# johannes-graeter/limo

Hardware: AMD Instinct MI355X
Metric: keyframe-BA window solves/sec (5 KF, ~2k landmarks) (higher is better)
Workload: dtype f64; 1 GPU; C2: KITTI-00-shaped windows, 5 keyframes x 2000 landmarks, LiDAR depth + ground plane, solveTrimmed schedule {2, trim 5%, <=100 LM iterations}; batch_windows_per_gpu=16384, distinct_windows_per_gpu=4096, observations_per_batch=144288124, depth_observations_per_batch=68405568, parallelism=single, converged=16328

## Files before the change

### include/limo_hip.h

```cpp
#ifndef LIMO_HIP_H_
#define LIMO_HIP_H_

#include <stddef.h>
#include <stdint.h>

#ifdef __cplusplus
extern "C" {
#endif

#define LIMO_ABI_VERSION 6

enum limo_fixation { LIMO_FIX_POSE = 0, LIMO_FIX_SCALE = 1, LIMO_FIX_NONE = 2 };

enum limo_status {
    LIMO_OK = 0,
    LIMO_ERR_INVALID = -1,
    LIMO_ERR_NOT_ENOUGH_KF = -2,
    LIMO_ERR_RUNTIME = -3,
    LIMO_ERR_NO_DEVICE = -4,
    LIMO_ERR_UNSUPPORTED = -5
};

enum limo_termination { LIMO_CONVERGENCE = 0, LIMO_NO_CONVERGENCE = 1, LIMO_FAILURE = 2 };

// ... 19 lines not shown
    const int32_t* obs_cam;
    const float* obs_u;
    const float* obs_v;
    const float* obs_d;
} limo_ba_window;

typedef struct limo_ba_options {
    double depth_thres;
    double reprojection_thres;
    double depth_quantile;
    double reprojection_quantile;
    int32_t num_trim_rounds;
    int32_t trim_solver_iterations;
    int32_t min_landmarks_for_trimming;
    int32_t minimum_number_residual_groups;
    int32_t max_num_iterations;
    double max_solver_time_sec;
    double function_tolerance;
    double gradient_tolerance;
    double parameter_tolerance;
    double initial_trust_region_radius;
    double max_trust_region_radius;
    double min_trust_region_radius;
    double min_lm_diagonal;
    double max_lm_diagonal;
    double min_relative_decrease;
    int32_t max_num_consecutive_invalid_steps;
    int32_t jacobi_scaling;
} limo_ba_options;

typedef struct limo_ba_report {
    int32_t termination;
    int32_t num_solves;
    int32_t iterations_total;
    int32_t iterations_final;
    int32_t successful_steps;
    int32_t n_depth_blocks;
    int32_t n_repr_blocks;
    int32_t n_gp_blocks;
    int32_t n_trimmed_landmarks;
    int32_t num_linearizations;
    double initial_cost;
    double final_cost;
    double time_sec;
} limo_ba_report;

typedef struct limo_ctx limo_ctx;
typedef struct limo_ba_batch limo_ba_batch;

int limo_abi_version(void);
int limo_ctx_create(int device, limo_ctx** out);
void limo_ctx_destroy(limo_ctx* ctx);
int limo_ctx_set_stream(limo_ctx* ctx, void* hip_stream);
const char* limo_last_error(const limo_ctx* ctx);
void* limo_host_alloc(size_t bytes);
void limo_host_free(void* p);

void limo_ba_default_options(limo_ba_options* out);

int limo_ba_solve(limo_ctx* ctx, limo_ba_window* window, const limo_ba_options* opts, limo_ba_report* report);

int limo_ba_batch_create(limo_ctx* ctx, int32_t n_windows, const limo_ba_window* windows, limo_ba_batch** out);
int limo_ba_batch_solve(limo_ba_batch* batch, const limo_ba_options* opts);
int limo_ba_batch_reset(limo_ba_batch* batch);
int limo_ba_batch_download(limo_ba_batch* batch, limo_ba_window* windows_out, limo_ba_report* reports);
void limo_ba_batch_destroy(limo_ba_batch* batch);
int limo_ba_batch_trimmed(limo_ba_batch* batch, int32_t window, uint8_t* removed);
int limo_ba_batch_kernel_stats(limo_ba_batch* batch, int reset, double* linearize_ms, int64_t* linearize_launches,
                               double* total_ms);
#define LIMO_KERNEL_LINEARIZE 0
#define LIMO_KERNEL_SCHUR 1
int limo_ba_batch_kernel_time(limo_ba_batch* batch, int kernel, double* ms, int64_t* launches);

#define LIMO_COMM_ID_BYTES 128
int limo_comm_unique_id(unsigned char id[LIMO_COMM_ID_BYTES]);
int limo_ctx_comm_init(limo_ctx* ctx, const unsigned char id[LIMO_COMM_ID_BYTES], int rank, int world);
typedef void (*limo_exchange_fn)(const double* send, double* recv, long long count, int kind, void* user);
int limo_ctx_comm_init_host(limo_ctx* ctx, limo_exchange_fn fn, void* user, int rank, int world);
int limo_ba_solve_sharded(limo_ctx* ctx, limo_ba_window* window, const limo_ba_options* opts, int n_shards,
                          limo_ba_report* report);
int limo_ctx_exchange_stats(limo_ctx* ctx, int64_t* stats3);
int64_t limo_ctx_coop_fallbacks(const limo_ctx* ctx);
int limo_ctx_last_solve_info(const limo_ctx* ctx, int64_t info[8]);

typedef struct limo_ba_iteration {
    int32_t solve;
    int32_t solve_kind;
    int32_t iteration;
    uint8_t step_is_valid, step_is_successful, pad[2];
    double cost;
    double cost_change, gradient_max_norm, step_norm, relative_decrease, trust_region_radius;
} limo_ba_iteration;
int limo_ctx_set_iteration_log(limo_ctx* ctx, int32_t on);
int limo_ba_batch_iteration_log(limo_ba_batch* batch, int32_t window, int32_t cap, limo_ba_iteration* out, int32_t* n);
int limo_ctx_last_iteration_log(limo_ctx* ctx, int32_t window, int32_t cap, limo_ba_iteration* out, int32_t* n);

int limo_ba_evaluate(limo_ctx* ctx, const limo_ba_window* window, const limo_ba_options* opts, int apply_loss,
                     double* cost, double* residuals, double* jac_pose, double* jac_lm, uint8_t* valid);

int limo_ba_evaluate_batch_time(limo_ctx* ctx, int32_t n_windows, const limo_ba_window* windows, const limo_ba_options* opts,
                                int32_t reps, double* device_ms);

typedef struct limo_speed_prior {
    double speed_weight;
    double dt_cur;
    double vel_prev[3];
    double pose_before[7];
} limo_speed_prior;
int limo_ba_adjust_pose_only(limo_ctx* ctx, limo_ba_window* window, const limo_speed_prior* prior,
                             const limo_ba_options* opts, limo_ba_report* report);

int limo_ba_batch_create_pose_only(limo_ctx* ctx, int32_t n_windows, const limo_ba_window* windows,
                                   const limo_speed_prior* priors, limo_ba_batch** out);
int limo_ba_adjust_pose_only_batch(limo_ctx* ctx, int32_t n_windows, limo_ba_window* windows, const limo_speed_prior* priors,
                                   const limo_ba_options* opts, limo_ba_report* reports);

int limo_ba_solve_fixed_landmarks(limo_ctx* ctx, limo_ba_window* window, const uint8_t* lm_fixed, const limo_ba_options* opts,
                                  limo_ba_report* report);
int limo_ba_batch_create_fixed_landmarks(limo_ctx* ctx, int32_t n_windows, const limo_ba_window* windows, const uint8_t* const* lm_fixed,
                                         limo_ba_batch** out);

enum limo_row_kind {
    LIMO_ROW_GROUND_HEIGHT = 0,
    LIMO_ROW_SCALE = 1,
    LIMO_ROW_NORMAL_DIFF = 2,
    LIMO_ROW_DIST_DIFF = 3,
    LIMO_ROW_PLANE_MOTION = 4,
    LIMO_ROW_GLOBAL_NORMAL = 5,
    LIMO_ROW_SPEED = 6
};
typedef struct limo_ba_row {
    int32_t kind;
    int32_t sub;
    int32_t kf[2];
    int32_t lm;
    int32_t fixed;
    double r;
    double cost;
    double jac_kf[2][10];
    double jac_lm[3];
} limo_ba_row;
int limo_ba_evaluate_rows(limo_ctx* ctx, const limo_ba_window* window, const limo_speed_prior* prior, int pose_only,
                          const limo_ba_options* opts, int32_t cap, limo_ba_row* rows, int32_t* n_rows);

typedef struct limo_ray {
    double pose_cam_origin[7];
    double f, cx, cy;
    float u, v, d;
    float pad;
} limo_ray;
int limo_landmark_init(limo_ctx* ctx, int32_t n, const int32_t* ray_off , const limo_ray* rays,
                       const uint8_t* use_depth , double* pos_out , uint8_t* ok );

int limo_trim_quantile(int32_t n, const int64_t* ids, const double* values, double quantile, int64_t* outliers_out);

typedef struct limo_depth_params {
    int32_t pixelarea_search_width;
    int32_t pixelarea_search_height;
    int32_t pixelarea_search_offset_x;
    int32_t pixelarea_search_offset_y;
    int32_t neighbors_count_min;
    int32_t do_use_histogram_segmentation;
    double histogram_segmentation_bin_width;
    int32_t histogram_segmentation_min_pointcount;
    int32_t treshold_depth_enabled;
    double treshold_depth_max;
// ... 99 lines not shown
```

### limo_amd/_ffi.py

```python
import ctypes as C
import os

_HERE = os.path.dirname(os.path.abspath(__file__))
LIB_PATH = os.environ.get("LIMO_HIP_LIB") or os.path.join(_HERE, "lib", "liblimo_hip.so")

LIMO_FIX_POSE, LIMO_FIX_SCALE, LIMO_FIX_NONE = 0, 1, 2
LIMO_OK, LIMO_ERR_INVALID, LIMO_ERR_NOT_ENOUGH_KF, LIMO_ERR_RUNTIME, LIMO_ERR_NO_DEVICE, LIMO_ERR_UNSUPPORTED = 0, -1, -2, -3, -4, -5
LIMO_CONVERGENCE, LIMO_NO_CONVERGENCE, LIMO_FAILURE = 0, 1, 2

c_double_p = C.POINTER(C.c_double)
c_float_p = C.POINTER(C.c_float)
c_int32_p = C.POINTER(C.c_int32)
c_int64_p = C.POINTER(C.c_int64)
c_uint8_p = C.POINTER(C.c_uint8)


class BaWindow(C.Structure):
    _fields_ = [
        ("n_kf", C.c_int32),
        ("n_cam", C.c_int32),
        ("n_lm", C.c_int32),
        ("n_obs", C.c_int32),
        ("kf_pose", c_double_p),
        ("kf_plane_dir", c_double_p),
# ... 173 lines not shown
        ("do_use_cut_behind_camera", C.c_int32),
        ("do_use_triangle_size_maximation", C.c_int32),
        ("do_check_triangleplanar_condition", C.c_int32),
        ("triangleplanar_crossnorm_treshold", C.c_double),
        ("viewray_plane_orthoganality_treshold", C.c_double),
        ("do_use_ransac_plane", C.c_int32),
        ("ransac_plane_distance_treshold", C.c_double),
        ("ransac_plane_min_z", C.c_double),
        ("ransac_plane_max_z", C.c_double),
        ("ransac_plane_max_iterations", C.c_int32),
        ("ransac_plane_probability", C.c_double),
        ("ransac_plane_use_refinement", C.c_int32),
        ("ransac_plane_refinement_treshold", C.c_double),
        ("ransac_plane_point_distance_treshold", C.c_double),
        ("plane_estimator_use_mestimator", C.c_int32),
        ("ransac_seed", C.c_uint64),
        ("neighbor_search_mode", C.c_int32),
        ("do_use_nearestNeighborSearch", C.c_int32),
        ("nnSearch_count", C.c_int32),
        ("do_use_radiusSearch", C.c_int32),
        ("radiusSearch_radius", C.c_double),
        ("radiusSearch_count_min", C.c_int32),
        ("do_use_depth_segmentation", C.c_int32),
        ("depth_segmentation_max_treshold_gradient", C.c_double),
        ("depth_segmentation_max_neighbor_distance", C.c_double),
        ("depth_segmentation_max_neighbor_distance_gradient", C.c_double),
        ("depth_segmentation_max_seedpoint_to_seedpoint_distance", C.c_double),
        ("depth_segmentation_max_seedpoint_to_seedpoint_distance_gradient", C.c_double),
        ("depth_segmentation_max_neighbor_to_seedpoint_distance", C.c_double),
        ("depth_segmentation_max_neighbor_to_seedpoint_distance_gradient", C.c_double),
        ("depth_segmentation_max_pointcount", C.c_int32),
        ("treshold_depth_mode", C.c_int32),
        ("treshold_depth_local_mode", C.c_int32),
        ("do_use_PCA", C.c_int32),
        ("pca_debug", C.c_double),
        ("pca_treshold_3_abs_min", C.c_double),
        ("pca_treshold_3_2_rel_max", C.c_double),
        ("pca_treshold_2_1_rel_min", C.c_double),
        ("ransac_plane_use_camx_treshold", C.c_int32),
        ("ransac_plane_treshold_camx", C.c_double),
        ("plane_estimator_use_triangle_maximation", C.c_int32),
        ("plane_estimator_use_leastsquares", C.c_int32),
        ("plane_estimator_z_x_min_relation", C.c_double),
        ("do_debug_singleFeatures", C.c_int32),
        ("do_publish_points", C.c_int32),
        ("do_depth_calc_statistics", C.c_int32),
    ]


(DEPTH_OK, DEPTH_NEIGHBOURS, DEPTH_HISTOGRAM, DEPTH_SEGMENT3, DEPTH_PLANAR, DEPTH_PARALLEL, DEPTH_GLOBAL, DEPTH_LOCAL, DEPTH_PCA,
 DEPTH_DEGENERATE) = range(10)
DEPTH_REASON_NAMES = ["OK", "NEIGHBOURS", "HISTOGRAM", "SEGMENT3", "PLANAR", "PARALLEL", "GLOBAL", "LOCAL", "PCA", "DEGENERATE"]


EXCHANGE_FN = C.CFUNCTYPE(None, C.POINTER(C.c_double), C.POINTER(C.c_double), C.c_longlong, C.c_int, C.c_void_p)

ABI_VERSION = 6

ABI_SYMBOLS = [
    "limo_abi_version",
    "limo_ctx_create",
    "limo_ctx_destroy",
    "limo_ctx_set_stream",
    "limo_last_error",
    "limo_host_alloc",
    "limo_host_free",
    "limo_ba_default_options",
    "limo_ba_solve",
    "limo_ba_batch_create",
    "limo_ba_batch_solve",
    "limo_ba_batch_reset",
    "limo_ba_batch_download",
    "limo_ba_batch_destroy",
    "limo_ba_batch_trimmed",
    "limo_ba_batch_kernel_stats",
    "limo_ba_batch_kernel_time",
    "limo_comm_unique_id",
    "limo_ctx_comm_init",
    "limo_ctx_comm_init_host",
    "limo_ba_solve_sharded",
    "limo_ctx_exchange_stats",
    "limo_ctx_coop_fallbacks",
    "limo_ctx_last_solve_info",
    "limo_ctx_set_iteration_log",
    "limo_ba_batch_iteration_log",
    "limo_ctx_last_iteration_log",
    "limo_ba_evaluate",
    "limo_ba_evaluate_batch_time",
    "limo_ba_evaluate_rows",
    "limo_ba_adjust_pose_only",
    "limo_ba_batch_create_pose_only",
    "limo_ba_adjust_pose_only_batch",
    "limo_ba_solve_fixed_landmarks",
    "limo_ba_batch_create_fixed_landmarks",
    "limo_landmark_init",
    "limo_trim_quantile",
    "limo_depth_default_params",
    "limo_depth_estimate",
    "limo_depth_estimate_begin",
    "limo_depth_estimate_end",
    "limo_depth_estimate_batch",
    "limo_depth_last_ground_plane",
    "limo_depth_last_reasons",
    "limo_depth_set_timing",
    "limo_depth_last_kernel_ms",
]

_lib = None


def load():
    global _lib
    if _lib is not None:
        return _lib
    if not os.path.exists(LIB_PATH):
        raise RuntimeError(
            "limo_amd: %s not found - run `python -c 'import __graft_entry__ as g; g.build()'` first. "
            "There is no CPU fallback for the product path." % LIB_PATH
        )
    try:
        import torch
    except ImportError:
        pass
    lib = C.CDLL(LIB_PATH, mode=C.RTLD_GLOBAL)
    vp = C.c_void_p
    lib.limo_abi_version.restype = C.c_int
    older = os.environ.get("LIMO_ALLOW_OLDER_ABI") == "1" and lib.limo_abi_version() < ABI_VERSION
    if lib.limo_abi_version() != ABI_VERSION and not older:
        raise RuntimeError("limo_amd: %s has ABI version %d, this binding needs %d - rebuild it (__graft_entry__.build())" % (LIB_PATH, lib.limo_abi_version(), ABI_VERSION))
    lib.limo_ctx_create.argtypes = [C.c_int, C.POINTER(vp)]
    lib.limo_ctx_destroy.argtypes = [vp]
    lib.limo_ctx_destroy.restype = None
    lib.limo_ctx_set_stream.argtypes = [vp, vp]
    lib.limo_last_error.argtypes = [vp]
    lib.limo_last_error.restype = C.c_char_p
    lib.limo_ba_default_options.argtypes = [C.POINTER(BaOptions)]
    lib.limo_ba_default_options.restype = None
    lib.limo_ba_solve.argtypes = [vp, C.POINTER(BaWindow), C.POINTER(BaOptions), C.POINTER(BaReport)]
    lib.limo_ba_batch_create.argtypes = [vp, C.c_int32, C.POINTER(BaWindow), C.POINTER(vp)]
    lib.limo_ba_batch_solve.argtypes = [vp, C.POINTER(BaOptions)]
    lib.limo_ba_batch_reset.argtypes = [vp]
    lib.limo_ba_batch_download.argtypes = [vp, C.POINTER(BaWindow), C.POINTER(BaReport)]
    lib.limo_ba_batch_destroy.argtypes = [vp]
    lib.limo_ba_batch_destroy.restype = None
    lib.limo_ba_batch_trimmed.argtypes = [vp, C.c_int32, c_uint8_p]
    lib.limo_ba_batch_kernel_stats.argtypes = [vp, C.c_int, c_double_p, c_int64_p, c_double_p]
    lib.limo_ba_batch_kernel_time.argtypes = [vp, C.c_int, c_double_p, c_int64_p]
    lib.limo_comm_unique_id.argtypes = [C.c_char_p]
    lib.limo_ctx_comm_init.argtypes = [vp, C.c_char_p, C.c_int, C.c_int]
    if not older:
        lib.limo_ctx_comm_init_host.argtypes = [vp, EXCHANGE_FN, C.c_void_p, C.c_int, C.c_int]
    lib.limo_ba_solve_sharded.argtypes = [vp, C.POINTER(BaWindow), C.POINTER(BaOptions), C.c_int, C.POINTER(BaReport)]
    lib.limo_ba_evaluate_batch_time.argtypes = [vp, C.c_int32, C.POINTER(BaWindow), C.POINTER(BaOptions), C.c_int32, C.POINTER(C.c_double)]
    lib.limo_ba_evaluate.argtypes = [
        vp,
        C.POINTER(BaWindow),
        C.POINTER(BaOptions),
        C.c_int,
        c_double_p,
        c_double_p,
        c_double_p,
        c_double_p,
        c_uint8_p,
    ]
    lib.limo_ba_evaluate_rows.argtypes = [vp, C.POINTER(BaWindow), C.POINTER(SpeedPrior), C.c_int, C.POINTER(BaOptions), C.c_int32, C.POINTER(BaRow), c_int32_p]
    lib.limo_ba_adjust_pose_only.argtypes = [
        vp,
        C.POINTER(BaWindow),
        C.POINTER(SpeedPrior),
        C.POINTER(BaOptions),
        C.POINTER(BaReport),
    ]
    if hasattr(lib, "limo_ba_batch_create_pose_only"):
        lib.limo_ba_batch_create_pose_only.argtypes = [vp, C.c_int32, C.POINTER(BaWindow), C.POINTER(SpeedPrior), C.POINTER(vp)]
        lib.limo_ba_adjust_pose_only_batch.argtypes = [vp, C.c_int32, C.POINTER(BaWindow), C.POINTER(SpeedPrior), C.POINTER(BaOptions), C.POINTER(BaReport)]
    if hasattr(lib, "limo_ba_solve_fixed_landmarks"):
        lib.limo_ba_solve_fixed_landmarks.argtypes = [vp, C.POINTER(BaWindow), c_uint8_p, C.POINTER(BaOptions), C.POINTER(BaReport)]
        lib.limo_ba_batch_create_fixed_landmarks.argtypes = [vp, C.c_int32, C.POINTER(BaWindow), C.POINTER(c_uint8_p), C.POINTER(vp)]
    lib.limo_landmark_init.argtypes = [vp, C.c_int32, c_int32_p, C.POINTER(Ray), c_uint8_p, c_double_p, c_uint8_p]
    lib.limo_trim_quantile.argtypes = [C.c_int32, c_int64_p, c_double_p, C.c_double, c_int64_p]
    lib.limo_depth_default_params.argtypes = [C.POINTER(DepthParams)]
    lib.limo_depth_default_params.restype = None
    lib.limo_depth_estimate.argtypes = [
        vp,
        c_float_p,
        C.c_size_t,
        c_double_p,
        C.c_double,
        C.c_double,
        C.c_double,
        C.c_int32,
        C.c_int32,
        c_float_p,
        C.c_size_t,
        c_uint8_p,
        C.POINTER(DepthParams),
        c_float_p,
    ]
    lib.limo_depth_estimate_begin.argtypes = lib.limo_depth_estimate.argtypes[:-1]
    lib.limo_depth_estimate_end.argtypes = [vp, c_float_p, C.c_size_t]
    lib.limo_host_alloc.argtypes = [C.c_size_t]
    lib.limo_host_alloc.restype = C.c_void_p
    lib.limo_host_free.argtypes = [C.c_void_p]
    lib.limo_host_free.restype = None
    lib.limo_depth_estimate_batch.argtypes = [vp, C.c_int32, C.POINTER(DepthFrame), c_double_p, C.c_double, C.c_double, C.c_double, C.c_int32, C.c_int32,
                                              C.POINTER(DepthParams), C.c_uint32]
    lib.limo_ctx_exchange_stats.argtypes = [vp, c_int64_p]
    lib.limo_ctx_coop_fallbacks.argtypes = [vp]
    lib.limo_ctx_coop_fallbacks.restype = C.c_int64
    if hasattr(lib, "limo_ctx_last_solve_info"):
        lib.limo_ctx_last_solve_info.argtypes = [vp, c_int64_p]
    if hasattr(lib, "limo_ctx_set_iteration_log"):
        lib.limo_ctx_set_iteration_log.argtypes = [vp, C.c_int32]
        lib.limo_ba_batch_iteration_log.argtypes = [vp, C.c_int32, C.c_int32, C.POINTER(BaIteration), c_int32_p]
        lib.limo_ctx_last_iteration_log.argtypes = [vp, C.c_int32, C.c_int32, C.POINTER(BaIteration), c_int32_p]
    lib.limo_depth_set_timing.argtypes = [vp, C.c_int32]
    lib.limo_depth_last_kernel_ms.argtypes = [vp, c_double_p]
    lib.limo_depth_last_ground_plane.argtypes = [vp, C.c_int32, c_double_p, c_int32_p]
    if not older:
        lib.limo_depth_last_reasons.argtypes = [vp, C.c_int32, c_uint8_p, C.c_size_t]
    _lib = lib
    return lib
```

### limo_amd/ba.py

```python
import ctypes as C

import numpy as np

from . import _ffi
from .window import struct_array


class LimoError(RuntimeError):
    pass


class NotEnoughKeyframes(LimoError):
    """BundleAdjusterKeyframes::NotEnoughKeyframesException (bundle_adjuster_keyframes.hpp:59-68)."""


def _check(rc, ctx=None, what=""):
    if rc == _ffi.LIMO_OK:
        return
    msg = ""
    if ctx is not None:
        msg = _ffi.load().limo_last_error(ctx).decode(errors="replace")
    if rc == _ffi.LIMO_ERR_NOT_ENOUGH_KF:
        raise NotEnoughKeyframes(msg or what)
    raise LimoError("%s failed: rc=%d %s" % (what, rc, msg))


class Context:
    def __init__(self, device=0, stream=None):
        self.lib = _ffi.load()
        self.device = device
        self.ptr = C.c_void_p()
        rc = self.lib.limo_ctx_create(device, C.byref(self.ptr))
        if rc != 0:
            raise LimoError("limo_ctx_create(device=%d) failed rc=%d (no gfx950 device? the product path has no CPU fallback)" % (device, rc))
        if stream is not None:
            self.set_stream(stream)

    def set_stream(self, stream):
        _check(self.lib.limo_ctx_set_stream(self.ptr, C.c_void_p(stream)), self.ptr, "limo_ctx_set_stream")

    def close(self):
        if self.ptr:
            self.lib.limo_ctx_destroy(self.ptr)
            self.ptr = C.c_void_p()

    def __del__(self):
        try:
            self.close()
        except Exception:
            pass

    def solve(self, window, opts, lm_fixed=None):
        s = window.as_struct()
        rep = _ffi.BaReport()
        if lm_fixed is not None:
            flags = fixed_flags(lm_fixed, window.n_lm)
            rc = self.lib.limo_ba_solve_fixed_landmarks(self.ptr, C.byref(s), flags.ctypes.data_as(_ffi.c_uint8_p), C.byref(opts), C.byref(rep))
            _check(rc, self.ptr, "limo_ba_solve_fixed_landmarks")
            return rep.as_dict()
        _check(self.lib.limo_ba_solve(self.ptr, C.byref(s), C.byref(opts), C.byref(rep)), self.ptr, "limo_ba_solve")
        return rep.as_dict()

    def solve_sharded(self, window, opts, n_shards):
        s = window.as_struct()
        rep = _ffi.BaReport()
        _check(self.lib.limo_ba_solve_sharded(self.ptr, C.byref(s), C.byref(opts), int(n_shards), C.byref(rep)), self.ptr, "limo_ba_solve_sharded")
        return rep.as_dict()

    def exchange_stats(self):
        st = (C.c_int64 * 3)()
        _check(self.lib.limo_ctx_exchange_stats(self.ptr, st), self.ptr, "limo_ctx_exchange_stats")
        return {"exchanges": int(st[0]), "bytes": int(st[1]), "iterations": int(st[2])}

    def coop_fallbacks(self):
        return int(self.lib.limo_ctx_coop_fallbacks(self.ptr))

    SOLVE_PATHS = {1: "WG", 2: "COOP", 3: "STREAMING", 4: "LOCKSTEP"}

    def last_solve_info(self):
        v = (C.c_int64 * 8)()
        _check(self.lib.limo_ctx_last_solve_info(self.ptr, v), self.ptr, "limo_ctx_last_solve_info")
        keys = ("recovered", "coop_G", "groups", "slots", "rounds", "pair_launches", "lin_variant")
        return dict({"path": self.SOLVE_PATHS.get(int(v[0]), "NONE")}, **{k: int(v[1 + i]) for i, k in enumerate(keys)})

    def set_iteration_log(self, on):
        _check(self.lib.limo_ctx_set_iteration_log(self.ptr, int(bool(on))), self.ptr, "limo_ctx_set_iteration_log")

    def last_iteration_log(self, window=0):
        return _read_iteration_log(lambda cap, out, n: self.lib.limo_ctx_last_iteration_log(self.ptr, int(window), cap, out, n), self.ptr,
                                   "limo_ctx_last_iteration_log")

    def comm_init(self, unique_id, rank, world):
        _check(self.lib.limo_ctx_comm_init(self.ptr, unique_id, int(rank), int(world)), self.ptr, "limo_ctx_comm_init")

    def comm_init_host(self, rank, world, allgather, allreduce):
        import numpy as np

        def _cb(send, recv, count, kind, _user):
            s = np.ctypeslib.as_array(send, shape=(count,))
            if kind == 0:
                allgather(s, np.ctypeslib.as_array(recv, shape=(world, count)))
            else:
                allreduce(s, np.ctypeslib.as_array(recv, shape=(count,)))

        self._xfn = _ffi.EXCHANGE_FN(_cb)
        _check(self.lib.limo_ctx_comm_init_host(self.ptr, self._xfn, None, int(rank), int(world)), self.ptr, "limo_ctx_comm_init_host")

    def comm_unique_id(self):
        buf = C.create_string_buffer(128)
        _check(self.lib.limo_comm_unique_id(buf), self.ptr, "limo_comm_unique_id")
        return buf.raw

    def landmark_init(self, ray_off, rays, use_depth):
        ray_off = np.ascontiguousarray(ray_off, np.int32)
        use_depth = np.ascontiguousarray(use_depth, np.uint8)
        n = len(use_depth)
        pos = np.zeros((n, 3))
        ok = np.zeros(n, np.uint8)
        rc = self.lib.limo_landmark_init(self.ptr, n, ray_off.ctypes.data_as(_ffi.c_int32_p), rays, use_depth.ctypes.data_as(_ffi.c_uint8_p),
                                         pos.ctypes.data_as(_ffi.c_double_p), ok.ctypes.data_as(_ffi.c_uint8_p))
        _check(rc, self.ptr, "limo_landmark_init")
        return pos, ok

    def adjust_pose_only(self, window, prior, opts):
        s = window.as_struct()
        rep = _ffi.BaReport()
        rc = self.lib.limo_ba_adjust_pose_only(self.ptr, C.byref(s), None if prior is None else C.byref(prior), C.byref(opts), C.byref(rep))
        _check(rc, self.ptr, "limo_ba_adjust_pose_only")
        return rep.as_dict()

    def adjust_pose_only_batch(self, windows, priors, opts):
        windows = list(windows)
        arr = struct_array(windows)
        reps = (_ffi.BaReport * max(1, len(windows)))()
        rc = self.lib.limo_ba_adjust_pose_only_batch(self.ptr, len(windows), arr, prior_array(priors, len(windows)), C.byref(opts), reps)
        _check(rc, self.ptr, "limo_ba_adjust_pose_only_batch")
        return [reps[i].as_dict() for i in range(len(windows))]

    def evaluate(self, window, opts, apply_loss=True):
        s = window.as_struct()
        M = window.n_obs
        cost = np.zeros(1)
        res = np.zeros((M, 3))
        jp = np.zeros((M, 3, 6))
        jl = np.zeros((M, 3, 3))
        valid = np.zeros(M, np.uint8)
        dp = lambda a: a.ctypes.data_as(_ffi.c_double_p)
        rc = self.lib.limo_ba_evaluate(self.ptr, C.byref(s), C.byref(opts), int(apply_loss), dp(cost), dp(res), dp(jp), dp(jl), valid.ctypes.data_as(_ffi.c_uint8_p))
        _check(rc, self.ptr, "limo_ba_evaluate")
        return float(cost[0]), res, jp, jl, valid


    def evaluate_rows(self, window, opts, pose_only=False, prior=None):
        s = window.as_struct()
        n = C.c_int32(0)
        cap = 64 + window.n_lm + 8 * window.n_kf
        rows = (_ffi.BaRow * cap)()
        rc = self.lib.limo_ba_evaluate_rows(self.ptr, C.byref(s), None if prior is None else C.byref(prior), int(pose_only), C.byref(opts), cap, rows, C.byref(n))
        _check(rc, self.ptr, "limo_ba_evaluate_rows")
        assert n.value <= cap
        return _ffi.rows_as_dicts(rows, n.value)


def _read_iteration_log(call, ctx_ptr, what):
    n = C.c_int32(0)
    _check(call(0, None, C.byref(n)), ctx_ptr, what)
# ... 231 lines not shown
```

### limo_amd/csrc/kba_batch_plan.hpp

```cpp
#pragma once
#include <algorithm>
#include <cstdint>
#include <cstdlib>
#include <vector>

#include "kba_items.hpp"
#include "kba_pack.hpp"

namespace kba {

struct PlanKernelSizes {
    int (*lean_lds)(int ncol);
    int (*wide_lds)(int nfp, int nc, int n_view);
    int lin_lds;
    int wide_waves;
    int trim_max_sort;
};

struct BatchPlan {
    bool any_fast = false, any_gen = false;
    int plain_tm = 1, plain_wpe = 4, gp_tm = 1, gp_wpe = 3;
    bool pair_ok = false;
    int wide_npw = 0;
    int plain_lds = 0, leangp_lds = 0, wide_lds = 0;
    int max_nc = 0;
    int asm_bytes = 0, solve_bytes = 0, trim_bytes = 0;
    int schur_wave_lds = 0;
    int onelaunch_lds = 0;
};

inline BatchPlan plan_batch(const PackedBatch& P, const PlanKernelSizes& ks) {
    BatchPlan p;
    int t_gen = 1, nfp_gen = 16, nc_gen = kCamSlots, nv_gen = 1, max_nfq = 0, max_nf = 0;
    for (const WinDesc& d : P.win) {
        p.max_nc = std::max(p.max_nc, (int)d.nc);
        if (d.schur_fast) {
            p.any_fast = true;
            max_nfq = std::max(max_nfq, (int)d.nfq);
            max_nf = std::max(max_nf, (int)d.nf);
        } else if (d.n_sblk > 0) {
            p.any_gen = true;
            t_gen = std::max(t_gen, d.nf_pad / 16);
            nfp_gen = std::max(nfp_gen, (int)d.nf_pad);
            nc_gen = std::max(nc_gen, (int)d.nc);
            nv_gen = std::max(nv_gen, (int)d.n_view);
        }
    }
    if (p.any_fast) {
        p.plain_tm = (max_nfq + 16) / 16 <= 1 ? 1 : 2;
        p.plain_wpe = p.plain_tm == 1 ? 4 : 3;
        p.plain_lds = ks.lean_lds(max_nfq + 1);
        p.gp_tm = std::min(3, (max_nf + 16) / 16);
        p.gp_wpe = p.gp_tm == 1 ? 3 : 2;
        p.leangp_lds = ks.lean_lds(max_nf + 1);
        p.pair_ok = p.plain_tm == 2 && p.gp_tm == 3;
    }
    if (p.any_gen) {
        const int tiles = t_gen * (t_gen + 1) / 2, npw = (tiles + ks.wide_waves - 1) / ks.wide_waves;
        p.wide_npw = npw <= 1 ? 1 : npw <= 3 ? 3 : npw <= 6 ? 6 : npw <= 12 ? 12 : -1;
        p.wide_lds = ks.wide_lds(nfp_gen, nc_gen, nv_gen);
    }
    {
        int nc_lds = kCamSlots, nf_lds = 1, nv_lds = 1;
        for (const WinDesc& d : P.win)
            if (d.cam_scr_off < 0) {
                nc_lds = std::max(nc_lds, (int)d.nc);
                nf_lds = std::max(nf_lds, (int)d.nf);
                nv_lds = std::max(nv_lds, (int)d.n_view);
            }
        p.asm_bytes = cam_assemble_scratch(nc_lds, kBlock, nv_lds) * (int)sizeof(double);
        p.solve_bytes = cam_solve_scratch(nc_lds, kBlock, nf_lds) * (int)sizeof(double);
    }
    int max_lm = 1, np2 = 1;
    for (const WinDesc& d : P.win) max_lm = std::max(max_lm, (int)d.n_lm);
    while (np2 < max_lm) np2 <<= 1;
    p.trim_bytes = np2 <= ks.trim_max_sort ? np2 * 12 + max_lm + 16 : 16;
    p.schur_wave_lds = (std::max(p.plain_lds, p.leangp_lds) + 15) / 16 * 16;
    p.onelaunch_lds = std::max(std::max(p.asm_bytes, p.solve_bytes), std::max(p.trim_bytes, ks.lin_lds));
    return p;
}

inline void build_sblk_list(const PackedBatch& P, const std::vector<int32_t>* windows, int span, int span_gp, int owner, std::vector<int32_t>& v,
                            int& n_plain, int& n_fgp) {
    v.clear();
    n_plain = n_fgp = 0;
    const int nw = windows ? (int)windows->size() : P.n_win;
    for (int cls = 0; cls < 3; ++cls) {
        for (int q = 0; q < nw; ++q) {
            const int w = windows ? (*windows)[q] : q;
            const WinDesc& d = P.win[w];
            if ((cls < 2) != (d.schur_fast != 0)) continue;
            auto groups = [&](int i0, int i1, int sp) {
                for (int i = i0; i < i1; i += sp)
                    if (owner < 0 || P.sblk_owner[d.sblk0 + i] == owner) v.push_back(d.sblk0 + i);
            };
            if (cls != 1) groups(0, d.n_sblk_plain, span);
            if (cls != 0) groups(d.n_sblk_plain, d.n_sblk, span_gp);
        }
        if (cls == 0) n_plain = (int)v.size();
        if (cls == 1) n_fgp = (int)v.size() - n_plain;
    }
}

constexpr int kCoopMaxWg = 256, kCoopMaxWin = 64;
constexpr int kWgMaxLblk = 8;
constexpr int kCoopRetryAfter = 64;

struct SolveSwitches {
    bool stream_min_set = false;
    int stream_min = 16;
    int coop_max_win = kCoopMaxWin;
    bool no_wg = false;
    bool no_coop = false;
    double coop_timeout_ms = 50.0;
    bool groups_set = false;
    int groups = 0;
};

inline SolveSwitches read_solve_switches() {
    SolveSwitches s;
    auto on = [](const char* name) {
        const char* e = std::getenv(name);
        return e && std::atoi(e) != 0;
    };
    if (const char* e = std::getenv("KBA_STREAM_MIN")) {
        s.stream_min_set = true;
        s.stream_min = std::atoi(e);
    }
    if (const char* e = std::getenv("KBA_COOP_MAX_WIN")) s.coop_max_win = std::min(std::atoi(e), kCoopMaxWg);
    s.no_wg = on("KBA_NO_WG_SOLVE");
    s.no_coop = on("KBA_NO_COOP_SOLVE");
    if (const char* e = std::getenv("KBA_COOP_TIMEOUT_MS")) s.coop_timeout_ms = std::atof(e);
    if (const char* e = std::getenv("KBA_GROUPS")) {
        s.groups_set = true;
        s.groups = std::atoi(e);
    }
    return s;
}

enum SolvePath { PATH_NONE = 0, PATH_WG = 1, PATH_COOP = 2, PATH_STREAMING = 3, PATH_LOCKSTEP = 4 };

struct SolveFacts {
    double max_solver_time_sec = -1.0;
    int shard_P = 1;
    bool pose_batch = false;
    bool pristine = true;
    int coop_strikes = 0, coop_benched = 0;
};
struct CoopGeometry {
    int G = 0, grid = 0;
};
struct SolveChoice {
    SolvePath path = PATH_LOCKSTEP;
    SolvePath fallback = PATH_LOCKSTEP;
    bool benched = false;
    CoopGeometry coop;
};

inline int plain_groups(const WinDesc& d, int span) { return (d.n_sblk_plain + span - 1) / span; }
inline int gp_groups(const WinDesc& d, int span_gp) { return (d.n_sblk - d.n_sblk_plain + span_gp - 1) / span_gp; }

inline bool wg_solve_applies(const PackedBatch& P, const BatchPlan& plan, const SolveSwitches& sw, int shard_P) {
    if (shard_P != 1 || P.evaluate_only || P.n_sblk != 0 || P.n_win < 1 || sw.no_wg) return false;
    for (const WinDesc& d : P.win)
        if (d.n_lblk > kWgMaxLblk) return false;
    return plan.onelaunch_lds <= kCamLdsCapBytes;
}

inline int coop_lds_bytes(const BatchPlan& plan) { return std::max(plan.onelaunch_lds, (kBlock / 64) * plan.schur_wave_lds); }

inline bool coop_solve_applies(const PackedBatch& P, const BatchPlan& plan, const SolveSwitches& sw, int shard_P, CoopGeometry& geo) {
    if (shard_P != 1 || P.evaluate_only || P.n_win < 1 || sw.no_coop) return false;
    int G = 1;
    for (const WinDesc& d : P.win) {
        if (!d.schur_fast || d.cam_scr_off >= 0 || d.nf_pad * d.nf_pad > kCoopRedStride) return false;
        const int tasks = plain_groups(d, kSchurSpan) + gp_groups(d, kSchurSpanGp);
        G = std::max(G, std::max((int)d.n_lblk, tasks ? 1 + (tasks + kBlock / 64 - 1) / (kBlock / 64) : 1));
    }
    G = std::min(G, 32);
    if (P.n_win > kCoopMaxWg || coop_lds_bytes(plan) > kCamLdsCapBytes) return false;
    const int per8 = ((int)P.n_win + 7) / 8;
    geo.G = std::max(1, std::min(G, kCoopMaxWg / (8 * per8)));
    geo.grid = 8 * geo.G * per8;
    return true;
}

inline SolveChoice choose_solve_path(const PackedBatch& P, const BatchPlan& plan, const SolveSwitches& sw, const SolveFacts& f) {
    SolveChoice ch;
    const bool pose_multi = f.pose_batch && P.n_win > 1;
    const bool can_stream = f.shard_P == 1 && f.max_solver_time_sec <= 0.0 && P.n_win >= sw.stream_min && !P.evaluate_only && !pose_multi;
    const bool one_launch = pose_multi || (!(sw.stream_min_set && can_stream) && P.n_win <= sw.coop_max_win);
    ch.path = ch.fallback = can_stream ? PATH_STREAMING : PATH_LOCKSTEP;
    if (!one_launch) return ch;
    if (wg_solve_applies(P, plan, sw, f.shard_P)) {
        ch.path = PATH_WG;
    } else if (!pose_multi && f.pristine && coop_solve_applies(P, plan, sw, f.shard_P, ch.coop)) {
        ch.benched = f.coop_strikes >= 3;
        if (!ch.benched || f.coop_benched + 1 >= kCoopRetryAfter) ch.path = PATH_COOP;
    }
    return ch;
}

struct SchurSpans {
    int plain = kSchurSpan, gp = kSchurSpanGp;
};
struct StreamGeometry {
    int n_slots = 0, n_groups = 0;
    int group_slots[4] = {0, 0, 0, 0};
    int mx[SL_COUNT] = {0};
};
inline StreamGeometry stream_geometry(const PackedBatch& P, const SchurSpans& spans, const SolveSwitches& sw) {
    StreamGeometry g;
    g.n_slots = std::min((int)P.n_win, std::max(1024, std::min(kSchedMaxSlots, (int)P.n_win / 4)));
    g.n_groups = sw.groups_set ? std::max(1, std::min(4, sw.groups)) : g.n_slots >= 4096 ? 3 : P.n_win >= 512 ? 2 : 1;
    for (int gi = 0; gi < g.n_groups; ++gi) g.group_slots[gi] = g.n_slots / g.n_groups + (gi < g.n_slots % g.n_groups ? 1 : 0);
    for (const WinDesc& d : P.win) {
        const int plg = plain_groups(d, spans.plain), gpg = gp_groups(d, spans.gp);
        g.mx[SL_LBLK] = std::max(g.mx[SL_LBLK], (int)d.n_lblk);
        g.mx[SL_TBLK] = std::max(g.mx[SL_TBLK], (int)d.n_blk);
// ... 12 lines not shown
```

### limo_amd/csrc/kba_items.hpp

```cpp
#pragma once
#include "kba_layout.hpp"
#include "kba_lm.hpp"
#include "kba_math.hpp"

#ifndef KBA_SYNC
#define KBA_SYNC() ((void)0)
#endif
#if defined(KBA_PROFILE_TICKS) && defined(__HIPCC__)
__device__ long long kba_ticks[2][24];
#endif
#if defined(KBA_PROFILE_TICKS) && defined(__HIP_DEVICE_COMPILE__)
#define KBA_TICK(n)                                                                   \
    do {                                                                              \
        if (w == 0 && (tid == 0 || tid == nt - 1)) kba_ticks[tid != 0][n] = clock64(); \
    } while (0)
#else
#define KBA_TICK(n) ((void)0)
#endif

namespace kba {

struct LinLane {
    double e[kLinPartial];
    int fail;
// ... 503 lines not shown
    const uint8_t* cm = bv.cmask + (int64_t)wd.cam0 + row0;
    if (cm[0]) {
        const double* pose = bv.pose + 7 * (int64_t)(wd.kf0 + kl);
        double R[9], M[9];
        bool have = false;
        for (int j = 0; j < wd.n_view; ++j) {
            if (vkl[j] != kl) continue;
            const int s = bv.lm_slot[(int64_t)j * bv.SL + gl];
            if (s < 0) continue;
            if (!have) {
                quat_R(pose, R);
                rot_tangent_from_R(R, quat_norm2_minus_1(pose), bv.lm + 3 * (int64_t)gl, M);
                have = true;
            }
            double Ft[9], c4[4];
            c4[0] = bv.obs_c[(int64_t)j * bv.SL + gl];
            c4[3] = bv.obs_c[obs_c_stride(bv) + (int64_t)j * bv.SL + gl];
            view_xy(bv.view_lin + (int64_t)kViewLin * (wd.view0 + j), bv.lm + 3 * (int64_t)gl, &c4[1], &c4[2]);
            ft_build(c4, bv.view_cam + 16 * (int64_t)(wd.view0 + j) + 4, Ft);
            schur_pose_block(Ft, R, M, lmk, sc + row0, Y);
        }
    }
    if (!with_plane) return;
    const int gg = bv.lm_gp[gl];
    if (gg < 0 || bv.gp_kf[gg] - wd.kf0 != kl) return;
    schur_gp_block(bv, gg, cm, lmk, sc + row0, Y);
}

KBA_HD void schur_load_lm(const BatchView& bv, int gl, double* lmk) {
#pragma unroll
    for (int i = 0; i < 6; ++i) lmk[i] = bv.lm_Li[i * bv.SL + gl];
}

KBA_HD int schur_plain_slabs(const WinDesc& wd, int span) { return (wd.n_sblk_plain + span - 1) / span; }
KBA_HD int schur_slabs(const WinDesc& wd, int span, int span_gp) {
    return schur_plain_slabs(wd, span) + (wd.n_sblk - wd.n_sblk_plain + span_gp - 1) / span_gp;
}
KBA_HD int schur_slab_of(const WinDesc& wd, int sb, int span, int span_gp) {
    const int i = sb - wd.sblk0;
    return i < wd.n_sblk_plain ? i / span : schur_plain_slabs(wd, span) + (i - wd.n_sblk_plain) / span_gp;
}
KBA_HD int schur_group_last(const WinDesc& wd, int sb, int span, int span_gp) {
    const int i = sb - wd.sblk0;
    const bool plain = i < wd.n_sblk_plain;
    const int end = plain ? wd.n_sblk_plain : wd.n_sblk, sp = plain ? span : span_gp;
    return wd.sblk0 + (i + sp < end ? i + sp : end) - 1;
}

KBA_HD int schur_need_count(int nf) { return nf * (nf + 1) / 2 + nf; }
KBA_HD int schur_need_pad(int nf) { return (schur_need_count(nf) + 31) / 32 * 32; }
KBA_HD void schur_need_decode(int i, int nf, int& ca, int& cb) {
    const int lda = nf + 1;
    ca = (int)(((2 * lda + 1) - sqrt((double)((2 * lda + 1) * (2 * lda + 1) - 8 * i))) * 0.5);
    while (ca > 0 && ca * lda - ca * (ca - 1) / 2 > i) --ca;
    while ((ca + 1) * lda - (ca + 1) * ca / 2 <= i) ++ca;
    cb = ca + (i - (ca * lda - ca * (ca - 1) / 2));
}
KBA_HD int schur_col(int i, int nfq);
KBA_HD int64_t schur_need_offset(int ca, int cb, int nf, int nfq, int nfp) {
    if (cb < nf) return (int64_t)schur_col(ca, nfq) * nfp + schur_col(cb, nfq);
    const int za = schur_col(ca, nfq);
    return za < nfq ? (int64_t)za * nfp + nfq : (int64_t)nfq * nfp + za;
}
KBA_HD void slab_reduce_entry(const BatchView& bv, int w, int n_shards, int i) {
    const WinDesc& wd = bv.win[w];
    const int64_t slab = (int64_t)wd.nf_pad * wd.nf_pad;
    int ca, cb;
    schur_need_decode(i, wd.nf, ca, cb);
    const double* sp = bv.S_part + wd.spart_off + schur_need_offset(ca, cb, wd.nf, wd.nfq, wd.nf_pad);
    double a = 0.0;
    const int q0 = (ca >= wd.nfq || (cb >= wd.nfq && cb < wd.nf)) ? wd.n_sblk_plain : 0;
    for (int q = q0; q < wd.n_sblk; ++q) a += sp[q * slab];
    bv.S_red[wd.sred_off / n_shards + i] = a;
}

KBA_HD int schur_col(int i, int nfq) {
    return i + (i >= nfq ? 1 : 0);
}

KBA_HD int schur_need_index(int n, int ca, int cb) { return ca * (n + 1) - ca * (ca - 1) / 2 + (cb - ca); }
KBA_HD int64_t slab_packed_base(int q, int n_plain, int nf, int nfq) {
    return q < n_plain ? (int64_t)q * schur_need_pad(nfq) : (int64_t)n_plain * schur_need_pad(nfq) + (int64_t)(q - n_plain) * schur_need_pad(nf);
}
KBA_HD SchurGroup schur_group_make(const WinDesc& wd, int w, int sb, int span, int span_gp, const int32_t* sblk_lm0, const int32_t* sblk_n,
                                   const int32_t* cslot) {
    SchurGroup g;
    const int sb_last = schur_group_last(wd, sb, span, span_gp);
    g.w = w;
    g.lm_first = sblk_lm0[sb];
    g.n_lm = sblk_lm0[sb_last] + sblk_n[sb_last] - g.lm_first;
    g.n_fk = wd.n_fk;
    g.nf = wd.nf, g.nfq = wd.nfq, g.nf_pad = wd.nf_pad;
    g.kf0 = wd.kf0, g.view0 = wd.view0, g.cam0 = wd.cam0;
    g.q_slab = schur_slab_of(wd, sb, span, span_gp);
    g.pad = 0;
    for (int k = 0; k < 4; ++k) {
        const bool on = k < wd.n_fk;
        g.kl[k] = on ? wd.fk[k] : -1;
        g.view[k] = on ? wd.fk_view[k] : -1;
        const int ci = on ? cslot[wd.cam0 + wd.fk[k] * kCamSlots] : -1;
        g.col0[k] = ci < 0 ? -1 : schur_col(ci, wd.nfq);
        g.pad2[k] = 0;
    }
    g.off_tile = wd.spart_off + (int64_t)g.q_slab * ((int64_t)wd.nf_pad * wd.nf_pad);
    g.off_packed = wd.spart_off + slab_packed_base(g.q_slab, schur_plain_slabs(wd, span), wd.nf, wd.nfq);
    return g;
}
KBA_HD int slab_packed_read(bool gp, int ca, int cb, int nf, int nfq) {
    if (gp) return schur_need_index(nf, ca, cb);
    if (ca >= nfq || (cb >= nfq && cb < nf)) return -1;
    return schur_need_index(nfq, ca, cb < nf ? cb : nfq);
}
KBA_HD int slab_packed_write(bool gp, int zr, int zc, int nf, int nfq) {
    const int n = gp ? nf : nfq;
    if (zr > zc || zc > n || (zr == nfq && zc == nfq)) return -1;
    if (zc == nfq) return schur_need_index(n, zr, n);
    if (zr == nfq) return schur_need_index(n, zc - 1, n);
    return schur_need_index(n, zr - (zr > nfq ? 1 : 0), zc - (zc > nfq ? 1 : 0));
}

struct LogProd {
    double m;
    int e;
};
KBA_HD void logprod_mul(LogProd& a, double x) {
    int ex;
    a.m *= frexp(x, &ex);
    a.e += ex;
}
KBA_HD double logprod_log(const LogProd& a) { return log(a.m) + static_cast<double>(a.e) * 0.69314718055994530942; }

KBA_HD void backsub_lane(const BatchView& bv, const SolveConsts& c, int w, int gl, double* part) {
    part[2] = part[3] = part[4] = part[6] = part[7] = 0.0;
    const int state = bv.lm_state[gl];
    const double* xp = bv.lm + 3 * (int64_t)gl;
    const double x[3] = {xp[0], xp[1], xp[2]};
    double xc[3] = {x[0], x[1], x[2]};
    if (state == 0) {
        double* o = bv.lm_c + 3 * (int64_t)gl;
        o[0] = xc[0];
        o[1] = xc[1];
        o[2] = xc[2];
        return;
    }
    const WinDesc& wd = bv.win[w];
    const int32_t* slot = bv.lm_slot + gl;
    const int n_view = wd.n_view;
    if (state == 1) {
        double a[3] = {0, 0, 0};
        const int j0 = wd.n_view_fixed0;
        const double* au_p = bv.obs_c;
        const double* sd_p = au_p + obs_c_stride(bv);
        int64_t r = (int64_t)j0 * bv.SL + gl;
        int s_cur = -1;
        double aun = 0.0, sdn = 0.0;
        if (j0 < n_view) {
            s_cur = bv.lm_slot[r];
            aun = au_p[r];
            sdn = sd_p[r];
        }
        for (int j = j0; j < n_view; ++j) {
            const bool have = s_cur >= 0;
            double c4[4];
            c4[0] = have ? aun : 0.0;
            c4[3] = have ? sdn : 0.0;
            r += j + 1 < n_view ? bv.SL : 0;
            s_cur = bv.lm_slot[r];
            aun = au_p[r];
            sdn = sd_p[r];
            const double* vs = bv.view_lin_c + (int64_t)kViewLin * (wd.view0 + j) + 28;
            const double* H = bv.view_lin + (int64_t)kViewLin * (wd.view0 + j);
            view_xy(H, x, &c4[1], &c4[2]);
            const double w0 = vs[0] * x[0] + vs[1] * x[1] + vs[2] * x[2] + vs[9];
            const double w1 = vs[3] * x[0] + vs[4] * x[1] + vs[5] * x[2] + vs[10];
            const double w2 = vs[6] * x[0] + vs[7] * x[1] + vs[8] * x[2] + vs[11];
            const double v0 = c4[0] * (c4[0] * (w0 - c4[1] * w2));
            const double v1 = c4[0] * (c4[0] * (w1 - c4[2] * w2));
            const double v2 = c4[3] * (c4[3] * w2) - c4[1] * v0 - c4[2] * v1;
            a[0] += H[0] * v0 + H[3] * v1 + H[6] * v2;
            a[1] += H[1] * v0 + H[4] * v1 + H[7] * v2;
            a[2] += H[2] * v0 + H[5] * v1 + H[8] * v2;
        }
        const int gg = bv.lm_gp[gl];
        if (gg >= 0) {
            const int gk = bv.gp_kf[gg];
            const double* dc = bv.delta_c + (int64_t)gk * kCamSlots;
            double q = 0.0;
            for (int k = 0; k < kCamSlots; ++k) q += bv.gp_F[k * bv.SG + gg] * dc[k];
            for (int cc = 0; cc < 3; ++cc) a[cc] += bv.gp_E[cc * bv.SG + gg] * q;
        }
        double Bt[6], t[3], V[6], g[3];
        for (int i = 0; i < 6; ++i) Bt[i] = bv.lm_Li[i * bv.SL + gl];
        for (int i = 0; i < 6; ++i) V[i] = bv.lm_V[i * bv.SL + gl];
        for (int i = 0; i < 3; ++i) g[i] = bv.lm_g[i * bv.SL + gl];
        lm_t_of(Bt, g, t);
        const double t0 = t[0] + Bt[0] * a[0];
        const double t1 = t[1] + Bt[1] * a[0] + Bt[2] * a[1];
        const double t2 = t[2] + Bt[3] * a[0] + Bt[4] * a[1] + Bt[5] * a[2];
        const double d0 = -(Bt[0] * t0 + Bt[1] * t1 + Bt[3] * t2);
        const double d1 = -(Bt[2] * t1 + Bt[4] * t2);
        const double d2 = -(Bt[5] * t2);
        xc[0] = x[0] + d0;
// ... 1160 lines not shown
```

### limo_amd/csrc/kba_kernels.hip

```cpp
#include <hip/hip_runtime.h>

#include <type_traits>

#define KBA_SYNC() __syncthreads()
#include "kba_items.hpp"

namespace kba {

__device__ __forceinline__ double wave_sum(double v) {
#pragma unroll
    for (int off = 32; off > 0; off >>= 1) v += __shfl_down(v, off, 64);
    return v;
}
__device__ __forceinline__ double wave_max(double v) {
#pragma unroll
    for (int off = 32; off > 0; off >>= 1) v = fmax(v, __shfl_down(v, off, 64));
    return v;
}

template <int N>
__device__ __forceinline__ void block_sum(const double* vals, double* lds , double* out_global) {
    const int lane = threadIdx.x & 63, wave = threadIdx.x >> 6;
#pragma unroll
    for (int i = 0; i < N; ++i) {
// ... 565 lines not shown
        const int nl = min(kSchurLm, n_lm_blk - l0);
        const int gl = lm_first + l0 + li;
        const bool live = li < nl && bv.lm_state[gl] == 1;
        double lmk[6];
        if (live) schur_load_lm(bv, gl, lmk);
        if (t < kSchurLm) {
            double t3[3] = {0.0, 0.0, 0.0};
            if (live) {
                const double g3[3] = {bv.lm_g[gl], bv.lm_g[bv.SL + gl], bv.lm_g[2 * bv.SL + gl]};
                lm_t_of(lmk, g3, t3);
            }
#pragma unroll
            for (int cc = 0; cc < 3; ++cc) Z[(3 * li + cc) * ld + nfq] = t3[cc];
        }
        for (int q = t >> 4; q < nfk; q += (64 * kWideWaves) >> 4) {
            const int kl = fk[q];
            double Y[3 * kCamSlots];
            if (live) {
                schur_pair_block(bv, wd, gl, kl, lmk, sc_s, vkl, tile_gp, Y);
            } else {
#pragma unroll
                for (int i = 0; i < 3 * kCamSlots; ++i) Y[i] = 0.0;
            }
#pragma unroll
            for (int a = 0; a < kCamSlots; ++a) {
                if (a < 6 || tile_gp) {
                    const int zc = zc_s[kl * kCamSlots + a];
                    if (zc >= 0) {
                        Z[(3 * li + 0) * ld + zc] = Y[a * 3 + 0];
                        Z[(3 * li + 1) * ld + zc] = Y[a * 3 + 1];
                        Z[(3 * li + 2) * ld + zc] = Y[a * 3 + 2];
                    }
                }
            }
        }
        __syncthreads();
        const double* zp = Z + (lane >> 4) * ld + (lane & 15);
#pragma unroll
        for (int j = 0; j < NPW; ++j) {
            const int ti = wave + kWideWaves * j;
            if (ti < n_tiles) {
                const int tr = ttr[ti], tc = ttc[ti];
                if (tc < Tt) {
#pragma unroll
                    for (int ks = 0; ks < 12; ++ks)
                        acc[j] = __builtin_amdgcn_mfma_f64_16x16x4f64(zp[ks * 4 * ld + 16 * tr], zp[ks * 4 * ld + 16 * tc], acc[j], 0, 0, 0);
                }
            }
        }
        __syncthreads();
    }
    double* out = bv.S_part + wd.spart_off + (int64_t)schur_slab_of(wd, sb, span, span_gp) * ((int64_t)nfp * nfp);
#pragma unroll
    for (int j = 0; j < NPW; ++j) {
        const int ti = wave + kWideWaves * j;
        if (ti < n_tiles) {
            const int tr = ttr[ti], tc = ttc[ti];
#pragma unroll
            for (int r = 0; r < 4; ++r)
                out[(tr * 16 + (lane >> 4) + 4 * r) * nfp + tc * 16 + (lane & 15)] = acc[j][r];
        }
    }
}

constexpr int kSpBatch = 4;
constexpr int kSpKf = 41;
constexpr int kSpRc = 9, kSpScale = 18, kSpQq1 = 28, kSpH = 29;

__host__ __device__ inline int schur_lean_ld(int ncol) { return ncol | 1; }
__host__ __device__ inline int schur_lean_lds_bytes(int ncol) {
    return (3 * kSchurLm * schur_lean_ld(ncol) + 16 + 4 * kSpKf) * (int)sizeof(double) + 4 * 12 * (int)sizeof(int);
}

template <bool COOP>
__device__ __forceinline__ void schur_wave_sync() {
    if constexpr (COOP) {
        __builtin_amdgcn_fence(__ATOMIC_RELEASE, "workgroup");
        __builtin_amdgcn_wave_barrier();
        __builtin_amdgcn_fence(__ATOMIC_ACQUIRE, "workgroup");
    } else {
        __syncthreads();
    }
}
template <int TM, bool GP, bool COOP>
__device__ __forceinline__ void schur_lean_group(const BatchView& bv, int sb, int span, int span_gp, int slab_packed, double* smem) {
    SchurGroup g;
    if (span == kSchurSpan && span_gp == kSchurSpanGp) {
        g = bv.sgrp[sb];
    } else {
        const int w = bv.sblk_win[sb];
        g = schur_group_make(bv.win[w], w, sb, span, span_gp, bv.sblk_lm0, bv.sblk_n, bv.cslot);
    }
    const int active = COOP ? 1 : __hip_atomic_load(&bv.st[g.w].active, __ATOMIC_RELAXED, __HIP_MEMORY_SCOPE_AGENT);
    const int nfq = g.nfq, nfp = g.nf_pad;
    const int ncol = GP ? g.nf + 1 : nfq + 1;
    const int ld = schur_lean_ld(ncol);
    const int Tt = (ncol + 15) / 16;
    constexpr bool kTT = !GP && TM == 2;
    const bool two_tile = kTT && Tt == 2;
    double* Z = smem;
    double* kc = Z + 3 * kSchurLm * ld + 16;
    int* zcs = reinterpret_cast<int*>(kc + 4 * kSpKf);
    const int lane = COOP ? (int)(threadIdx.x & 63) : (int)threadIdx.x, li = lane & 15, kq = lane >> 4;
    const int n_fk = g.n_fk;
    const int my_kl = kq == 0 ? g.kl[0] : kq == 1 ? g.kl[1] : kq == 2 ? g.kl[2] : g.kl[3];
    const int my_view = kq == 0 ? g.view[0] : kq == 1 ? g.view[1] : kq == 2 ? g.view[2] : g.view[3];
    const int my_col0 = kq == 0 ? g.col0[0] : kq == 1 ? g.col0[1] : kq == 2 ? g.col0[2] : g.col0[3];
    const bool have = my_col0 >= 0;
    const int slot0 = g.cam0 + (my_kl >= 0 ? my_kl : 0) * kCamSlots;
    const int32_t* my_slots = bv.lm_slot + (int64_t)(my_view >= 0 ? my_view - g.view0 : 0) * bv.SL;
    const int lm_first = g.lm_first, n_lm_blk = g.n_lm;

    constexpr int NT = (!GP && TM == 2) ? 2 : TM * (TM + 1) / 2;
    v4f64 acc[NT];
#pragma unroll
    for (int i = 0; i < NT; ++i) acc[i] = (v4f64){0.0, 0.0, 0.0, 0.0};

    auto index_issue = [&](int l0, int& st, int& slot, int& gr) {
        const int i = l0 + li < n_lm_blk ? l0 + li : n_lm_blk - 1;
        const int gl = lm_first + i;
        st = bv.lm_state[gl];
        slot = my_slots[gl];
        gr = -1;
        if constexpr (GP) gr = bv.lm_gp[gl];
    };
    auto index_kf = [&](int gr) {
        if constexpr (GP) return bv.gp_kf[gr >= 0 ? gr : 0];
        return 0;
    };
    double c4[4], p[3], Bt[6], g3[3], gE[3], gF[kCamSlots];
    const bool has_pair = have && my_view >= 0;
    const bool want_g = kq == 0 || two_tile;
    const double* my_au = bv.obs_c + (int64_t)(my_view >= 0 ? my_view - g.view0 : 0) * bv.SL;
    const double* my_sd = my_au + obs_c_stride(bv);
    auto data_issue = [&](int l0) {
        const int gl = lm_first + (l0 + li < n_lm_blk ? l0 + li : n_lm_blk - 1);
        if (has_pair) {
            c4[0] = my_au[gl];
            c4[3] = my_sd[gl];
#pragma unroll
            for (int i = 0; i < 3; ++i) p[i] = bv.lm[3 * (int64_t)gl + i];
        }
        if (has_pair || want_g || (GP && have)) {
#pragma unroll
            for (int i = 0; i < 6; ++i) Bt[i] = bv.lm_Li[i * bv.SL + gl];
        }
        if (want_g) {
#pragma unroll
            for (int i = 0; i < 3; ++i) g3[i] = bv.lm_g[i * bv.SL + gl];
        }
    };
    auto gp_issue = [&](bool on, int gg) {
        if constexpr (GP) {
            if (on) {
#pragma unroll
                for (int i = 0; i < 3; ++i) gE[i] = bv.gp_E[i * bv.SG + gg];
#pragma unroll
                for (int i = 0; i < kCamSlots; ++i) gF[i] = bv.gp_F[i * bv.SG + gg];
            }
        }
    };
    bool live = false, seen = false, att = false;
    auto predicates = [&](int l0, int st, int slot, int gg, int kf) {
        const bool in = l0 + li < n_lm_blk;
        live = in && st == 1;
        seen = live && has_pair && slot >= 0;
        att = GP && live && have && gg >= 0 && kf - g.kf0 == my_kl;
    };
    int c_st, c_slot, c_gg, c_kf = 0;
    int n_st = 0, n_slot = -1, n_gg = -1, n_kf = 0;
    {
        index_issue(0, c_st, c_slot, c_gg);
        if constexpr (GP) index_issue(kSchurLm, n_st, n_slot, n_gg);
        const double* vl = bv.view_lin + (int64_t)kViewLin * (my_view >= 0 ? my_view : 0);
        const double v0 = vl[li], v1 = vl[16 + li], v2 = vl[32 + li];
        const int my_slot = slot0 + (li < kCamSlots ? li : 0);
        const double sc = bv.scale_c[my_slot];
        const int ci = bv.cslot[my_slot];
        data_issue(0);
        if constexpr (GP) {
            c_kf = index_kf(c_gg);
            n_kf = index_kf(n_gg);
            gp_issue(have && li < n_lm_blk && c_gg >= 0, c_gg);
        }
        if (!active) return;
        if (kq < n_fk) {
            double* mine_w = kc + kq * kSpKf;
            const bool vw = my_view >= 0;
            mine_w[li < 12 ? kSpH + li : kSpRc + li - 12] = vw ? v0 : 0.0;
            if (li < 5) mine_w[kSpRc + 4 + li] = vw ? v1 : 0.0;
            if (li >= 5 && li < 15) mine_w[li == 14 ? kSpQq1 : li - 5] = vw ? v2 : 0.0;
            if (li < kCamSlots) {
                mine_w[kSpScale + li] = sc;
                zcs[kq * 12 + li] = ci < 0 ? -1 : schur_col(ci, nfq);
            }
        }
        if (lane < 16) Z[3 * kSchurLm * ld + lane] = 0.0;
        schur_wave_sync<COOP>();
    }
    const double* mine = kc + (kq < n_fk ? kq : 0) * kSpKf;
    constexpr int NS = GP ? kCamSlots : 6;
    double yt[6] = {0.0, 0.0, 0.0, 0.0, 0.0, 0.0};
    const int mq = li < 8 ? li : li + 8;
    for (int l0 = 0; l0 < n_lm_blk; l0 += kSchurLm) {
        predicates(l0, c_st, c_slot, c_gg, c_kf);
        double t3[3] = {0.0, 0.0, 0.0};
        if (live && (kq == 0 || two_tile)) lm_t_of(Bt, g3, t3);
        if (kq == 0 && !two_tile) {
#pragma unroll
            for (int cc = 0; cc < 3; ++cc) Z[(3 * li + cc) * ld + nfq] = live ? t3[cc] : 0.0;
        }
        if (have) {
            double Y[3 * NS];
#pragma unroll
            for (int i = 0; i < 3 * NS; ++i) Y[i] = 0.0;
            if (seen) {
                double M[9], Ft[9];
                rot_tangent_from_R(mine, mine[kSpQq1], p, M);
                view_xy(mine + kSpH, p, &c4[1], &c4[2]);
                ft_build(c4, mine + kSpRc, Ft);
                schur_pose_block<true>(Ft, mine, M, Bt, mine + kSpScale, Y);
                if (two_tile) {
#pragma unroll
                    for (int a = 0; a < 6; ++a) yt[a] += Y[a * 3 + 0] * t3[0] + Y[a * 3 + 1] * t3[1] + Y[a * 3 + 2] * t3[2];
                }
            }
            if constexpr (GP) {
                if (att) {
                    const double y0 = gE[0] * Bt[0], y1 = gE[0] * Bt[1] + gE[1] * Bt[2], y2 = gE[0] * Bt[3] + gE[1] * Bt[4] + gE[2] * Bt[5];
#pragma unroll
                    for (int a = 0; a < kCamSlots; ++a) {
                        const double fa = zcs[kq * 12 + a] >= 0 ? gF[a] * mine[kSpScale + a] : 0.0;
                        Y[a * 3 + 0] += fa * y0;
                        Y[a * 3 + 1] += fa * y1;
                        Y[a * 3 + 2] += fa * y2;
                    }
                }
            }
            double* zrow = Z + 3 * li * ld + zcs[kq * 12];
#pragma unroll
            for (int a = 0; a < 6; ++a) {
                zrow[a] = Y[a * 3 + 0];
                zrow[ld + a] = Y[a * 3 + 1];
                zrow[2 * ld + a] = Y[a * 3 + 2];
            }
            if constexpr (GP) {
#pragma unroll
                for (int a = 6; a < kCamSlots; ++a) {
                    const int zc = zcs[kq * 12 + a];
                    if (zc >= 0) {
                        Z[(3 * li + 0) * ld + zc] = Y[a * 3 + 0];
                        Z[(3 * li + 1) * ld + zc] = Y[a * 3 + 1];
                        Z[(3 * li + 2) * ld + zc] = Y[a * 3 + 2];
                    }
                }
            }
        }
        if (l0 + kSchurLm < n_lm_blk) {
            const int l1 = l0 + kSchurLm;
            if constexpr (GP) {
                c_st = n_st, c_slot = n_slot, c_gg = n_gg, c_kf = n_kf;
                index_issue(l1 + kSchurLm, n_st, n_slot, n_gg);
                n_kf = index_kf(n_gg);
                data_issue(l1);
                gp_issue(have && l1 + li < n_lm_blk && c_st == 1 && c_gg >= 0 && c_kf - g.kf0 == my_kl, c_gg);
            } else {
                index_issue(l1, c_st, c_slot, c_gg);
                data_issue(l1);
            }
        }
        schur_wave_sync<COOP>();
        const double* zp = Z + kq * ld + li;
        if (TM == 1 || Tt == 1) {
#pragma unroll
            for (int h = 0; h < 12; h += kSpBatch) {
                double pa[kSpBatch];
#pragma unroll
                for (int j = 0; j < kSpBatch; ++j) pa[j] = zp[(h + j) * 4 * ld];
#pragma unroll
                for (int j = 0; j < kSpBatch; ++j) acc[0] = __builtin_amdgcn_mfma_f64_16x16x4f64(pa[j], pa[j], acc[0], 0, 0, 0);
            }
        } else if (kTT) {
            if constexpr (kTT) {
                constexpr int kB = 3;
#pragma unroll
                for (int h = 0; h < 12; h += kB) {
                    double pa[kB], pb[kB], pq[kB];
#pragma unroll
                    for (int j = 0; j < kB; ++j) {
                        pa[j] = zp[(h + j) * 4 * ld];
                        pb[j] = zp[(h + j) * 4 * ld + 8];
                        pq[j] = Z[((h + j) * 4 + kq) * ld + mq];
                    }
#pragma unroll
                    for (int j = 0; j < kB; ++j) {
                        acc[0] = __builtin_amdgcn_mfma_f64_16x16x4f64(pa[j], pb[j], acc[0], 0, 0, 0);
                        acc[1] = __builtin_amdgcn_mfma_f64_16x16x4f64(pq[j], pq[j], acc[1], 0, 0, 0);
                    }
                }
            }
        } else if (TM == 2 || Tt == 2) {
            if constexpr (TM >= 2 && !kTT) {
                constexpr int i11 = TM;
#pragma unroll
                for (int h = 0; h < 12; h += kSpBatch) {
                    double pa[kSpBatch], pb[kSpBatch];
#pragma unroll
                    for (int j = 0; j < kSpBatch; ++j) {
                        pa[j] = zp[(h + j) * 4 * ld];
                        pb[j] = zp[(h + j) * 4 * ld + 16];
                    }
#pragma unroll
                    for (int j = 0; j < kSpBatch; ++j) {
                        acc[0] = __builtin_amdgcn_mfma_f64_16x16x4f64(pa[j], pa[j], acc[0], 0, 0, 0);
                        acc[1] = __builtin_amdgcn_mfma_f64_16x16x4f64(pa[j], pb[j], acc[1], 0, 0, 0);
                        acc[i11] = __builtin_amdgcn_mfma_f64_16x16x4f64(pb[j], pb[j], acc[i11], 0, 0, 0);
                    }
                }
            }
        } else {
            if constexpr (TM >= 3) {
#pragma unroll
                for (int h = 0; h < 12; h += 2) {
                    double pn[2][3];
#pragma unroll
                    for (int j = 0; j < 2; ++j)
#pragma unroll
                        for (int t = 0; t < 3; ++t) pn[j][t] = zp[(h + j) * 4 * ld + 16 * t];
#pragma unroll
                    for (int j = 0; j < 2; ++j) {
                        acc[0] = __builtin_amdgcn_mfma_f64_16x16x4f64(pn[j][0], pn[j][0], acc[0], 0, 0, 0);
                        acc[1] = __builtin_amdgcn_mfma_f64_16x16x4f64(pn[j][0], pn[j][1], acc[1], 0, 0, 0);
                        acc[2] = __builtin_amdgcn_mfma_f64_16x16x4f64(pn[j][0], pn[j][2], acc[2], 0, 0, 0);
                        acc[3] = __builtin_amdgcn_mfma_f64_16x16x4f64(pn[j][1], pn[j][1], acc[3], 0, 0, 0);
                        acc[4] = __builtin_amdgcn_mfma_f64_16x16x4f64(pn[j][1], pn[j][2], acc[4], 0, 0, 0);
                        acc[5] = __builtin_amdgcn_mfma_f64_16x16x4f64(pn[j][2], pn[j][2], acc[5], 0, 0, 0);
                    }
                }
            }
        }
        schur_wave_sync<COOP>();
    }
    const bool packed = !COOP && slab_packed != 0;
    double* out = bv.S_part + (packed ? g.off_packed : g.off_tile);
    const int T = nfp / 16;
    if (two_tile && packed) {
#pragma unroll
        for (int r = 0; r < 4; ++r) {
            const int row = kq + 4 * r;
            {
                const int col = 8 + li;
                if (row <= col && col < nfq) out[slab_packed_write(false, row, col, g.nf, nfq)] = acc[0][r];
            }
            {
                const int a = row < 8 ? row : row + 8, b = mq;
                if (a <= b && b < nfq && !(a < 8 && b >= 16)) out[slab_packed_write(false, a, b, g.nf, nfq)] = acc[1][r];
            }
        }
        if (have) {
#pragma unroll
            for (int a = 0; a < 6; ++a) {
                double v = yt[a];
                v += __shfl_xor(v, 1, 64);
                v += __shfl_xor(v, 2, 64);
                v += __shfl_xor(v, 4, 64);
                v += __shfl_xor(v, 8, 64);
                if (li == 0) out[slab_packed_write(false, zcs[kq * 12] + a, nfq, g.nf, nfq)] = v;
            }
        }
        return;
    }
    if (two_tile) {
        double* St = Z;
        for (int i = lane; i < 1024; i += 64) St[i] = 0.0;
        schur_wave_sync<COOP>();
#pragma unroll
        for (int r = 0; r < 4; ++r) {
            const int row = kq + 4 * r;
            {
                const int col = 8 + li;
                if (row <= col && col < nfq) St[row * 32 + col] = acc[0][r];
            }
            {
                const int a = row < 8 ? row : row + 8, b = mq;
                if (a <= b && b < nfq && !(a < 8 && b >= 16)) St[a * 32 + b] = acc[1][r];
            }
        }
        if (have) {
#pragma unroll
            for (int a = 0; a < 6; ++a) {
                double v = yt[a];
                v += __shfl_xor(v, 1, 64);
                v += __shfl_xor(v, 2, 64);
                v += __shfl_xor(v, 4, 64);
                v += __shfl_xor(v, 8, 64);
                if (li == 0) St[(zcs[kq * 12] + a) * 32 + nfq] = v;
            }
        }
        schur_wave_sync<COOP>();
        for (int tc = 0; tc < (T < 2 ? T : 2); ++tc)
            for (int tr = 0; tr <= tc; ++tr) {
#pragma unroll
                for (int r = 0; r < 4; ++r) {
                    const int row = tr * 16 + kq + 4 * r, col = tc * 16 + li;
                    out[row * nfp + col] = St[row * 32 + col];
                }
            }
        return;
    }
    if constexpr (kTT) {
#pragma unroll
        for (int r = 0; r < 4; ++r) {
            const int row = kq + 4 * r, col = li;
            if (packed) {
                const int k = slab_packed_write(false, row, col, g.nf, nfq);
                if (k >= 0) out[k] = acc[0][r];
            } else {
                out[row * nfp + col] = (row < ncol && col < ncol) ? acc[0][r] : 0.0;
            }
        }
    } else {
        int idx = 0;
#pragma unroll
        for (int tr = 0; tr < TM; ++tr)
#pragma unroll
            for (int tc = tr; tc < TM; ++tc) {
                if (tc < T) {
#pragma unroll
                    for (int r = 0; r < 4; ++r) {
                        const int row = tr * 16 + kq + 4 * r, col = tc * 16 + li;
                        if (packed) {
                            const int k = slab_packed_write(GP, row, col, g.nf, nfq);
                            if (k >= 0) out[k] = acc[idx][r];
                        } else {
                            out[row * nfp + col] = (row < ncol && col < ncol) ? acc[idx][r] : 0.0;
                        }
                    }
                }
                ++idx;
            }
        if constexpr (GP) {
            if (!packed)
                for (int tc = TM; tc < T; ++tc)
                    for (int tr = 0; tr <= tc; ++tr) {
#pragma unroll
                        for (int r = 0; r < 4; ++r) out[(tr * 16 + kq + 4 * r) * nfp + tc * 16 + li] = 0.0;
                    }
        }
    }
}
template <int TM, bool GP, int WAVES>
__global__ __launch_bounds__(64) __attribute__((amdgpu_waves_per_eu(WAVES, WAVES))) void k_schur_lean(
    BatchView bv, const int32_t* wl, int span, int span_gp, int slab_packed) {
    const int sb = wl_at(bv, wl, blockIdx.x);
    if (sb < 0) return;
    extern __shared__ __attribute__((aligned(16))) double smem[];
    schur_lean_group<TM, GP, false>(bv, sb, span, span_gp, slab_packed, smem);
}

template <int TMP, int TMG>
__global__ __launch_bounds__(64) void k_schur_lean_pair(BatchView bv, const int32_t* wl_plain, int n_plain_cap, const int32_t* wl_gp, int span, int span_gp, int slab_packed) {
    extern __shared__ __attribute__((aligned(16))) double smem[];
    if ((int)blockIdx.x < n_plain_cap) {
        const int sb = wl_at(bv, wl_plain, blockIdx.x);
        if (sb >= 0) schur_lean_group<TMP, false, false>(bv, sb, span, span_gp, slab_packed, smem);
    } else {
        const int sb = wl_at(bv, wl_gp, blockIdx.x - n_plain_cap);
        if (sb >= 0) schur_lean_group<TMG, true, false>(bv, sb, span, span_gp, slab_packed, smem);
    }
}

__global__ __launch_bounds__(kBlock) __attribute__((amdgpu_waves_per_eu(3, 3))) void k_cam_assemble(BatchView bv, SolveConsts c, const int32_t* wl) {
    const int w = wl_at(bv, wl, blockIdx.x);
    if (w < 0) return;
    WinState& st = bv.st[w];
    extern __shared__ __attribute__((aligned(16))) double smem[];
    if (st.active && st.need_lin) {
        const int64_t so = bv.win[w].cam_scr_off;
        if (so >= 0)
            cam_assemble(bv, c, w, threadIdx.x, blockDim.x, bv.cam_scratch + so);
        else
            cam_assemble(bv, c, w, threadIdx.x, blockDim.x, smem);
        __syncthreads();
#ifdef KBA_PROFILE_TICKS
        if (w == 0 && threadIdx.x == 0)
            for (int l = 0; l < 2; ++l)
                printf("[ticks cam_assemble %s lane] observation blocks %lld, ground-plane rows %lld, regulariser rows %lld, their sums %lld, mask + store %lld, reductions %lld\n",
                       l ? "last" : "first", kba_ticks[l][1] - kba_ticks[l][0], kba_ticks[l][2] - kba_ticks[l][1], kba_ticks[l][3] - kba_ticks[l][2],
                       kba_ticks[l][4] - kba_ticks[l][3], kba_ticks[l][5] - kba_ticks[l][4], kba_ticks[l][6] - kba_ticks[l][5]);
#endif
        if (threadIdx.x == 0) lm_decide_lin(st, bv.red[w], bv.reg_cost[2 * w + 1], c);
    }
    __syncthreads();
    if (threadIdx.x == 0 && !bv.counted) {
        if (st.active) atomicAdd(bv.n_active, 1);
        __threadfence();
        if (atomicAdd(bv.n_active + 1, 1) == (int)gridDim.x - 1) {
            __threadfence();
            const int total = atomicAdd(bv.n_active, 0);
            bv.n_active[0] = 0;
            bv.n_active[1] = 0;
            *(volatile int32_t*)bv.n_active_host = total;
            __threadfence_system();
        }
    }
}

__global__ __launch_bounds__(kBlock) void k_cam_solve(BatchView bv, SolveConsts c, const int32_t* wl) {
    const int w = wl_at(bv, wl, blockIdx.x);
    if (w < 0) return;
    if (!bv.st[w].active) return;
    extern __shared__ __attribute__((aligned(16))) double smem[];
    __shared__ int flag;
    const int64_t so = bv.win[w].cam_scr_off;
    if (so >= 0)
        cam_solve(bv, c, w, threadIdx.x, blockDim.x, bv.cam_scratch + so, &flag);
    else
        cam_solve(bv, c, w, threadIdx.x, blockDim.x, smem, &flag);
#ifdef KBA_PROFILE_TICKS
    __syncthreads();
    if (w == 0 && threadIdx.x == 0)
        for (int l = 0; l < 2; ++l)
            printf("[ticks cam_solve %s lane] slab sum %lld, cholesky %lld, back-substitution %lld, step %lld, reduction %lld\n", l ? "last" : "first",
                   kba_ticks[l][9] - kba_ticks[l][8], kba_ticks[l][10] - kba_ticks[l][9], kba_ticks[l][11] - kba_ticks[l][10],
                   kba_ticks[l][12] - kba_ticks[l][11], kba_ticks[l][13] - kba_ticks[l][12]);
#endif
}

__global__ __launch_bounds__(64) void k_step_decide(BatchView bv, SolveConsts c, const int32_t* wl) {
    const int w = wl_at(bv, wl, blockIdx.x);
    if (w < 0) return;
    if (!bv.st[w].active) return;
    __shared__ double red[64];
    reduce_step(bv, w, threadIdx.x, blockDim.x, red);
    __syncthreads();
    if (threadIdx.x == 0) lm_decide_step(bv.st[w], bv.red[w], c);
    __syncthreads();
    if (bv.st[w].accept) accept_keyframes(bv, bv.win[w], threadIdx.x, blockDim.x);
}

__global__ __launch_bounds__(kBlock) void k_after_step(BatchView bv, SolveConsts c, const int32_t* wl) {
    const int b = wl_at(bv, wl, blockIdx.x);
    if (b < 0) return;
    lm_damp_block(bv, c, b);
}

__global__ __launch_bounds__(kBlock) void k_trim_residual(BatchView bv, double* plane_rep, double* plane_dep, const int32_t* wl) {
    const int b = wl_at(bv, wl, blockIdx.x);
    if (b < 0) return;
    const int w = bv.view_win[bv.blk_view[b]];
    if (!bv.win[w].do_trim) return;
// ... 667 lines not shown
```

### limo_amd/csrc/kba_layout.hpp

```cpp
#pragma once
#include <stddef.h>
#include <stdint.h>

#include "../../include/limo_hip.h"

namespace kba {

constexpr int kMaxKf = 20;
constexpr int kMaxViews = 64;
constexpr int kViewLin = 64;
constexpr int kCamSlots = 10;
constexpr int kMaxNc = kMaxKf * kCamSlots;
constexpr int kBlock = 256;
constexpr int kObsPerLane = 4;
constexpr int kObsBlock = kBlock * kObsPerLane;
constexpr int kSchurLm = 16;
constexpr int kSchurLmPerBlock = 64;
constexpr int kSchurSpan = 2, kSchurSpanGp = 1;
constexpr int kMaxRegRows = 1 + (kMaxKf - 1) * 5 + 3 * kMaxKf;

constexpr int kGpRed = 65;
constexpr int kLinPartial = 28;
constexpr int kLinFixedCost = 26;
constexpr int kLinWaves = 4;

struct EvalChunk {
    int32_t base, view, o0, o1, dep0, pad;
};

struct WinDesc {
    int32_t kf0, n_kf;
    int32_t lm0, n_lm;
    int32_t view0, n_view;
    int32_t obs0, n_obs;
    int32_t blk0, n_blk;
    int32_t lblk0, n_lblk;
    int32_t gp0, n_gp;
    int32_t sblk0, n_sblk;
    int32_t n_sblk_plain;
    int32_t schur_fast, n_fk;
    int32_t fk[4];
    int32_t fk_view[4];
    int32_t nc, nc_pad;
    int32_t nf, nf_pad;
    int32_t nfq;
    int32_t lm_gp0;
    int32_t cam0;
    int32_t reg0;
    int32_t has_scale_reg, has_gp_reg;
    int32_t n_depth, n_repr;
    int32_t do_trim;
    int32_t pose_only;
    int32_t n_view_fixed0;
    int32_t n_lm_const;
    double scale_w, scale_s0;
    double speed_w, speed_dt, speed_vel[3], speed_Rb[9], speed_tb[3];
    int64_t hcc_off;
    int64_t spart_off;
    int64_t sred_off;
    int64_t xlv_off;
    int64_t lvpart_off;
    int64_t cam_scr_off;
};

struct alignas(128) SchurGroup {
    int32_t w;
    int32_t lm_first, n_lm;
    int32_t n_fk;
    int32_t nf, nfq, nf_pad;
    int32_t kf0, view0, cam0;
    int32_t q_slab;
    int32_t pad;
    int32_t kl[4];
    int32_t view[4];
    int32_t col0[4];
    int64_t off_tile;
    int64_t off_packed;
    int32_t pad2[4];
};
static_assert(sizeof(SchurGroup) == 128, "one cache line per record");

struct WinState {
    int32_t active, need_lin, first, accept;
    int32_t iter, max_iter, term, invalid_run;
    int32_t in_phase;
    int32_t compute_scale;
    int32_t n_success, n_unsuccess;
    int32_t acc_solves, acc_iters, acc_success, last_iters;
    int32_t n_trimmed, acc_lin;
    int32_t phase, trim_round;
    int32_t redamp;
    int32_t log_kind;
    double radius, decrease_factor;
    double x_cost, x_norm, fixed_cost;
    double solve_initial_cost, solve_final_cost;
    double first_initial_cost;
    double rho_pending, xnorm_pending, cost_pending;
    double gmax;
    double step_pending, dcost_pending;
    limo_ba_iteration* log;
    int32_t log_n, log_cap;
    int32_t log_solve;
    int32_t log_si;
};

struct WinRed {
    double lin_cost;
    double gmax;
    double xnorm2;
    double mcc;
    double step2;
    double cand2;
    double cand_cost;
    int32_t lin_fail, chol_fail, cand_fail;
    int32_t no_variable;
};

enum SchedPhase { PH_IDLE = 0, PH_TRIM_SOLVE = 1, PH_RETRY = 2, PH_TRIM = 3, PH_FINAL = 4, PH_DONE = 5 };

enum SchedList { SL_LBLK = 0, SL_SPLAIN, SL_SFGP, SL_SGEN, SL_WIN, SL_TBLK, SL_TLBLK, SL_TWIN, SL_COUNT };
constexpr int kSchedThreads = 1024;
constexpr int kSchedSlotsPerLane = 4;
constexpr int kSchedMaxSlots = kSchedThreads * kSchedSlotsPerLane;
constexpr int kCoopRedStride = 64 * 64;

struct SolveConsts {
    double a_rep, a_dep;
    double inv_a_rep2, inv_a_dep2;
    double function_tolerance, gradient_tolerance, parameter_tolerance;
    double initial_radius, max_radius, min_radius, min_lm_diagonal, max_lm_diagonal, min_relative_decrease;
    int32_t max_invalid, jacobi_scaling;
    double depth_quantile, reprojection_quantile;
    int32_t min_groups, pad;
    int32_t schur_span;
    int32_t schur_span_gp;
    int32_t num_trim_rounds, trim_iters, max_iters;
    int32_t schur_nslab;
    int32_t schur_packed;
    int32_t slab_packed;
};

struct BatchView {
    int32_t n_win, TK, TL, TO, TV, TG, n_blk, n_lblk, n_sblk, Vmax;
    int64_t SO, SL, SG;
    const WinDesc* win;
    WinState* st;
    WinRed* red;
    double *pose, *pdir, *pdist, *lm;
    double *pose_c, *pdir_c, *pdist_c, *lm_c;
    const int32_t* kf_win;
    const int32_t* kf_blk0;
    const int32_t* kf_nblk;
    const int32_t* kf_gp0;
    const int32_t* kf_ngp;
    uint8_t* cmask;
    uint8_t* cpresent;
    const int32_t* cslot;
    const int32_t* lm_win;
    const int32_t* lm_id;
    const double* lm_weight;
    uint8_t* lm_state;
    const int32_t* lm_gp;
    const int32_t* lm_slot;
// ... 87 lines not shown
```

### limo_amd/csrc/kba_pack.cpp

```cpp
#include "kba_pack.hpp"

#include <algorithm>
#include <atomic>
#include <chrono>
#include <cmath>
#include <cstdio>
#include <cstdlib>
#include <cstring>
#include <condition_variable>
#include <functional>
#include <limits>
#include <mutex>
#include <numeric>
#include <thread>
#include <pthread.h>
#include <unistd.h>
#include <exception>

#include "kba_items.hpp"

namespace kba {

namespace {
thread_local PackArena* t_pack_arena = nullptr;
// ... 648 lines not shown
    std::vector<Base> base(n);
    {
        Base run{0, 0, 0, 0};
        for (int w = 0; w < n; ++w) {
            Local& L = locals[w];
            if (L.rc != LIMO_OK) {
                err = po.per_window_prior ? "window " + std::to_string(w) + ": " + L.err : L.err;
                return L.rc;
            }
            base[w] = run;
            run.blk += (int)L.blk_view.size();
            run.lblk += (int)L.lblk_win.size();
            run.sblk += (int)L.sblk_win.size();
            run.gp += (int)L.gp_lm.size();
            WinDesc& d = P.win[w];
            d.blk0 += base[w].blk;
            d.lblk0 += base[w].lblk;
            d.sblk0 += base[w].sblk;
            d.gp0 += base[w].gp;
            d.hcc_off = P.hcc_total;
            P.hcc_total += (int64_t)d.nc * d.nc;
            d.spart_off = P.spart_total;
            P.spart_total += (int64_t)d.n_sblk * ((int64_t)d.nf_pad * d.nf_pad);
            d.sred_off = P.sred_total;
            if (P.n_shards > 1) P.sred_total += (int64_t)P.n_shards * schur_need_pad(d.nf);
            d.xlv_off = P.xlv_total;
            P.xlv_total += (int64_t)d.n_view * kLinPartial;
            d.lvpart_off = P.lvpart_total;
            P.lvpart_total += (int64_t)d.n_lblk * d.n_view * kLinPartial;
            {
                const int need = std::max(cam_assemble_scratch(d.nc, kBlock, d.n_view), cam_solve_scratch(d.nc, kBlock));
                d.cam_scr_off = -1;
                if (need * (int)sizeof(double) > kCamLdsCapBytes) {
                    d.cam_scr_off = P.camscr_total;
                    P.camscr_total += need;
                }
            }
        }
        for (auto* v : {&P.blk_view, &P.blk_obs0, &P.blk_n, &P.blk_owner}) v->resize(run.blk);
        for (auto* v : {&P.lblk_win, &P.lblk_lm0, &P.lblk_n, &P.lblk_owner}) v->resize(run.lblk);
        for (auto* v : {&P.sblk_win, &P.sblk_lm0, &P.sblk_n, &P.sblk_owner}) v->resize(run.sblk);
        for (auto* v : {&P.gp_lm, &P.gp_kf, &P.gp_owner}) v->resize(run.gp);
        P.gp_w.resize(run.gp);
    }
    for_windows([&](int w) {
        Local& L = locals[w];
        const WinDesc& d = P.win[w];
        const Base& bs = base[w];
        for (int k = d.kf0; k < d.kf0 + d.n_kf; ++k) {
            if (P.kf_nblk[k]) P.kf_blk0[k] += bs.blk;
            if (P.kf_ngp[k]) P.kf_gp0[k] += bs.gp;
        }
        for (int l = d.lm0; l < d.lm0 + d.n_lm; ++l)
            if (P.lm_gp[l] >= 0) P.lm_gp[l] += bs.gp;
        auto put = [](auto& dst, const auto& src, int at) { std::copy(src.begin(), src.end(), dst.begin() + at); };
        put(P.blk_view, L.blk_view, bs.blk);
        put(P.blk_obs0, L.blk_obs0, bs.blk);
        put(P.blk_n, L.blk_n, bs.blk);
        put(P.blk_owner, L.blk_owner, bs.blk);
        put(P.lblk_win, L.lblk_win, bs.lblk);
        put(P.lblk_lm0, L.lblk_lm0, bs.lblk);
        put(P.lblk_n, L.lblk_n, bs.lblk);
        put(P.lblk_owner, L.lblk_owner, bs.lblk);
        put(P.sblk_win, L.sblk_win, bs.sblk);
        put(P.sblk_lm0, L.sblk_lm0, bs.sblk);
        put(P.sblk_n, L.sblk_n, bs.sblk);
        put(P.sblk_owner, L.sblk_owner, bs.sblk);
        put(P.gp_lm, L.gp_lm, bs.gp);
        put(P.gp_kf, L.gp_kf, bs.gp);
        put(P.gp_w, L.gp_w, bs.gp);
        put(P.gp_owner, L.gp_owner, bs.gp);
        L = Local();
    });
    if (std::getenv("KBA_PACK_TRACE"))
        std::fprintf(stderr, "[kba] pack: views + sizes %.1f ms, arrays %.1f ms, fill %.1f ms, merge %.1f ms\n", std::chrono::duration<double, std::milli>(t_p0b - t_p0).count(),
                     std::chrono::duration<double, std::milli>(t_p1 - t_p0b).count(), std::chrono::duration<double, std::milli>(t_p2 - t_p1).count(),
                     std::chrono::duration<double, std::milli>(std::chrono::steady_clock::now() - t_p2).count());
    P.TG = (int)P.gp_lm.size();
    P.SG = pad64(std::max(1, P.TG));
    P.n_blk = (int)P.blk_view.size();
    P.n_lblk = (int)P.lblk_win.size();
    P.n_sblk = (int)P.sblk_win.size();
    P.sgrp.assign((size_t)P.n_sblk, SchurGroup{});
    for_windows([&](int w) {
        const WinDesc& d = P.win[w];
        if (!d.schur_fast) return;
        for (int sb = d.sblk0; sb < d.sblk0 + d.n_sblk; ++sb)
            P.sgrp[sb] = schur_group_make(d, w, sb, kSchurSpan, kSchurSpanGp, P.sblk_lm0.data(), P.sblk_n.data(), P.cslot.data());
    });
    if (P.evaluate_only) {
        P.echunk.clear();
        P.obs_rank.assign((size_t)std::max(1, P.TO), -1);
        std::vector<int32_t> before((size_t)P.TO + 1, 0);
        for (int o = 0; o < P.TO; ++o) {
            const bool dep = P.obs_d[o] > 0.0f;
            if (dep) P.obs_rank[o] = before[o];
            before[o + 1] = before[o] + (dep ? 1 : 0);
        }
        P.TD = before[P.TO];
        P.SD = pad64(std::max(1, P.TD)) + 64;
        for (int b = 0; b < P.n_blk; ++b) {
            const int o0 = P.blk_obs0[b], o1 = o0 + P.blk_n[b];
            for (int a = o0; a < o1; a += 64) {
                EvalChunk ch;
                ch.base = a;
                ch.view = P.blk_view[b];
                ch.o0 = o0;
                ch.o1 = o1;
                ch.dep0 = before[a];
                ch.pad = 0;
                P.echunk.push_back(ch);
            }
        }
        P.n_echunk = (int)P.echunk.size();
    }
    return LIMO_OK;
}

void run_schedule(Executor& ex, const limo_ba_options& o) {
    using Clock = std::chrono::steady_clock;
    auto run_solve = [&](int max_iter, int select) {
        ex.solve_init(max_iter, select);
        const auto t0 = Clock::now();
        for (;;) {
            ex.linearize();
            if (ex.active_count() == 0) break;
            if (o.max_solver_time_sec > 0.0 &&
                std::chrono::duration<double>(Clock::now() - t0).count() >= o.max_solver_time_sec) {
                ex.expire(0);
                break;
            }
            ex.step();
        }
    };
    for (int r = 0; r < o.num_trim_rounds; ++r) {
        run_solve(o.trim_solver_iterations, 1);
        run_solve(3 * o.trim_solver_iterations, 2);
        ex.trim();
    }
    run_solve(o.max_num_iterations, 0);
}

}
```

### limo_amd/csrc/kba_pack.hpp

```cpp
#pragma once
#include <memory>
#include <string>
#include <type_traits>
#include <utility>
#include <vector>

#include "kba_layout.hpp"

namespace kba {

struct PackArena {
    char* base = nullptr;
    size_t cap = 0, used = 0;
    size_t wanted = 0;
};
constexpr size_t kPackArenaMin = 64u << 10;
void pack_arena_lend(PackArena* a);
void pack_arena_register(const void* base, size_t cap, bool add);
bool pack_arena_owns(const void* p);
void* pack_arena_take(size_t bytes);
struct PackArenaLend {
    explicit PackArenaLend(PackArena* a) { pack_arena_lend(a); }
    ~PackArenaLend() { pack_arena_lend(nullptr); }
    PackArenaLend(const PackArenaLend&) = delete;
    PackArenaLend& operator=(const PackArenaLend&) = delete;
};

template <typename T>
struct default_init_allocator : std::allocator<T> {
    template <typename U>
    struct rebind {
        using other = default_init_allocator<U>;
    };
    T* allocate(size_t n) {
        const size_t bytes = n * sizeof(T);
        if (bytes >= kPackArenaMin)
            if (void* p = pack_arena_take(bytes)) return static_cast<T*>(p);
        return static_cast<T*>(::operator new(bytes));
    }
    void deallocate(T* p, size_t) noexcept {
        if (pack_arena_owns(p)) return;
        ::operator delete(p);
    }
    template <typename U>
    void construct(U* p) noexcept(std::is_nothrow_default_constructible<U>::value) {
        ::new (static_cast<void*>(p)) U;
    }
    template <typename U, typename... Args>
    void construct(U* p, Args&&... args) {
        ::new (static_cast<void*>(p)) U(std::forward<Args>(args)...);
    }
};
template <typename T>
using uvec = std::vector<T, default_init_allocator<T>>;

struct PackedBatch {
    int32_t n_win = 0, TK = 0, TL = 0, TO = 0, TV = 0, TG = 0, n_blk = 0, n_lblk = 0, n_sblk = 0, Vmax = 0;
    int64_t SO = 0, SL = 0, SG = 0;
    int64_t SD = 0;
    int32_t TD = 0;
    int64_t hcc_total = 0, spart_total = 0, sred_total = 0, camscr_total = 0, lvpart_total = 0, xlv_total = 0;
    bool evaluate_only = false;
    int32_t n_shards = 1;
    std::vector<int32_t> blk_owner, lblk_owner, sblk_owner, gp_owner;
    std::vector<WinDesc> win;
    std::vector<double> pose, pdir, pdist;
    uvec<double> lm;
    std::vector<int32_t> kf_win, kf_blk0, kf_nblk, kf_gp0, kf_ngp;
    std::vector<uint8_t> cmask, cpresent;
    std::vector<int32_t> cslot;
    uvec<int32_t> lm_gp;
    uvec<int32_t> lm_win, lm_slot;
    uvec<int32_t> lm_id;
    uvec<double> lm_weight;
    uvec<uint8_t> lm_state;
    std::vector<int32_t> view_kf, view_win;
    std::vector<double> view_cam;
    std::vector<int32_t> blk_view, blk_obs0, blk_n;
    std::vector<EvalChunk> echunk;
    int32_t n_echunk = 0;
    std::vector<int32_t> obs_rank;
    uvec<int32_t> obs_lm;
    uvec<float> obs_u, obs_v, obs_d;
    uvec<int32_t> obs_src;
    std::vector<int32_t> lblk_win, lblk_lm0, lblk_n, sblk_win, sblk_lm0, sblk_n;
    std::vector<SchurGroup> sgrp;
    std::vector<int32_t> gp_lm, gp_kf;
    std::vector<double> gp_w;
};

struct PackOptions {
    bool pose_only = false;
    bool evaluate_only = false;
    const limo_speed_prior* prior = nullptr;
    int shards = 1;
    bool per_window_prior = false;
    const limo_speed_prior* window_priors = nullptr;
    const uint8_t* const* lm_fixed = nullptr;
};

int pack_windows(int32_t n, const limo_ba_window* windows, const limo_ba_options& opts, const PackOptions& po,
                 PackedBatch& out, std::string& err);

SolveConsts make_consts(const limo_ba_options& o);

struct Executor {
    virtual ~Executor() {}
    virtual void solve_init(int max_iter, int select) = 0;
    virtual void linearize() = 0;
    virtual int active_count() = 0;
    virtual void step() = 0;
    virtual void trim() = 0;
    virtual void expire(int) {}
};

void run_schedule(Executor& ex, const limo_ba_options& o);

}
```

### limo_amd/csrc/limo_ctx.hpp

```cpp
#pragma once
#include <hip/hip_runtime.h>

#include <algorithm>
#include <cstdlib>
#include <map>
#include <string>
#include <vector>

#include "kba_pack.hpp"

struct PinnedBuf {
    void* p = nullptr;
    size_t cap = 0;
    hipError_t ensure(size_t bytes, size_t min_bytes = 0, size_t max_bytes = ~size_t(0)) {
        if (cap >= bytes) return hipSuccess;
        release();
        const size_t want = std::min(max_bytes, std::max(bytes, min_bytes));
        const hipError_t e = hipHostMalloc(&p, want);
        if (e == hipSuccess)
            cap = want;
        else
            p = nullptr;
        return e;
    }
    void release() {
        if (p) (void)hipHostFree(p);
        p = nullptr;
        cap = 0;
    }
};

struct limo_ctx {
    int device = 0;
    hipStream_t stream = nullptr;
    hipStream_t own = nullptr;
    std::string err;
    void* depth_ws = nullptr;
    void (*depth_ws_free)(void*) = nullptr;
    void* comm = nullptr;
    int comm_rank = 0, comm_world = 1;
    void (*xfn)(const double* send, double* recv, long long count, int kind, void* user) = nullptr;
    void* xuser = nullptr;
    PinnedBuf xhost;
    bool has_transport() const { return comm != nullptr || xfn != nullptr; }
    long long exchange_stats[3] = {0, 0, 0};
    long long coop_fallbacks = 0;
    int coop_strikes = 0;
    int coop_benched = 0;
    long long last_solve_info[8] = {0, 0, 0, 0, 0, 0, 0, 0};
    bool iteration_log = false;
    std::vector<limo_ba_iteration> last_log;
    std::vector<int32_t> last_log_n;
    std::vector<size_t> last_log_off;
    static constexpr int kPoolPerClass = 4;
    static constexpr size_t kPoolMaxBlock = 32u << 20;
    std::map<size_t, std::vector<void*>> pool, host_pool;
    PinnedBuf staging;
    PinnedBuf pack_arena;
    size_t pack_arena_wanted = 0;
    bool pack_arena_busy = false;
    static constexpr size_t kPackArenaMax = size_t(1) << 30;
    PinnedBuf staging_big;
    static constexpr size_t kBigStageMax = 512u << 20;

    static constexpr size_t kLargeStep = 64u << 20;
    static constexpr size_t kPoolLargeBytes = size_t(16) << 30;
    size_t pooled_large = 0;
    static size_t size_class(size_t bytes) {
        if (bytes > kPoolMaxBlock) return (bytes + kLargeStep - 1) / kLargeStep * kLargeStep;
        size_t c = 256;
        while (c < bytes) c <<= 1;
        return c;
    }
    hipError_t pool_alloc(void** p, size_t bytes) {
        const size_t c = size_class(bytes);
        static const bool no_reuse = std::getenv("KBA_NO_POOL") != nullptr;
        if (no_reuse) return hipMalloc(p, c);
        auto it = pool.find(c);
        if (it != pool.end() && !it->second.empty()) {
            *p = it->second.back();
            it->second.pop_back();
            if (bytes > kPoolMaxBlock) pooled_large -= c;
            return hipSuccess;
        }
        hipError_t e = hipMalloc(p, c);
        while (e == hipErrorOutOfMemory && trim_largest()) {
            (void)hipGetLastError();
            e = hipMalloc(p, c);
        }
        return e;
    }
    bool trim_largest() {
        for (auto it = pool.rbegin(); it != pool.rend(); ++it) {
            if (it->second.empty()) continue;
            (void)hipFree(it->second.back());
            it->second.pop_back();
            if (it->first > kPoolMaxBlock) pooled_large -= it->first;
            return true;
        }
        return false;
    }
    void pool_free(void* p, size_t bytes) {
        const size_t c = size_class(bytes);
        auto& v = pool[c];
        static const bool no_reuse = std::getenv("KBA_NO_POOL") != nullptr;
        const bool large = bytes > kPoolMaxBlock;
        if (!no_reuse && (large ? (v.empty() && pooled_large + c <= kPoolLargeBytes) : (int)v.size() < kPoolPerClass)) {
            v.push_back(p);
            if (large) pooled_large += c;
        } else {
            (void)hipFree(p);
        }
    }
    hipError_t host_alloc(void** p, size_t bytes) {
        const size_t c = size_class(bytes);
        auto it = host_pool.find(c);
        if (it != host_pool.end() && !it->second.empty()) {
            *p = it->second.back();
            it->second.pop_back();
            return hipSuccess;
        }
        return hipHostMalloc(p, c);
    }
    void host_free(void* p, size_t bytes) {
        auto& v = host_pool[size_class(bytes)];
        if ((int)v.size() < kPoolPerClass && bytes <= kPoolMaxBlock)
            v.push_back(p);
        else
            (void)hipHostFree(p);
    }
    void pool_release() {
        for (auto& kv : host_pool)
// ... 14 lines not shown
```

### limo_amd/csrc/limo_hip.hip

```cpp
#include <hip/hip_runtime.h>
#include <rccl/rccl.h>

#include <algorithm>
#include <chrono>
#include <cmath>
#include <cstdio>
#include <cstring>
#include <atomic>
#include <memory>
#include <new>
#include <string>
#include <thread>
#include <vector>

#include "kba_kernels.hip"

#include "kba_batch_plan.hpp"
#include "kba_buffers.hpp"
#include "kba_rows.hpp"

using namespace kba;

#include "limo_ctx.hpp"

#define HIP_TRY(ctx, expr)                                                                       \
    do {                                                                                         \
        hipError_t e__ = (expr);                                                                 \
        if (e__ != hipSuccess) {                                                                 \
            (ctx)->err = std::string(#expr) + ": " + hipGetErrorString(e__);                     \
            return LIMO_ERR_RUNTIME;                                                             \
        }                                                                                        \
    } while (0)

namespace {

inline int cdiv(int64_t a, int64_t b) {
    return (int)((a + b - 1) / b);
}

struct EventPair {
    hipEvent_t a, b;
    int kernel;
};

}

struct limo_ba_batch : Executor {
    limo_ctx* ctx = nullptr;
    PackedBatch P;
    bool holds_pack_arena = false;
    bool pose_batch = false;
    BatchView bv;
    SolveConsts c;
    limo_ba_options opts;
    std::vector<std::pair<void*, size_t>> allocs;
    double *d_plane_rep = nullptr, *d_plane_dep = nullptr;
    double *d_pose0 = nullptr, *d_pdir0 = nullptr, *d_pdist0 = nullptr, *d_lm0 = nullptr;
    uint8_t* d_lm_state0 = nullptr;
    std::vector<WinState> st0;
    int32_t* h_active = nullptr;
    int32_t* d_h_active = nullptr;
    size_t h_flags_bytes = 0;
    hipEvent_t act_ev[4] = {nullptr, nullptr, nullptr, nullptr};
    int it_no = 0;
    struct WorkLists {
        const int32_t *blk = nullptr, *lblk = nullptr, *sblk = nullptr, *win = nullptr;
        int n_blk = 0, n_lblk = 0, n_sblk_plain = 0, n_sblk_fgp = 0, n_sblk = 0, n_win = 0;
    };
    struct ViewLists {
        WorkLists full, cur;
        int owner = -1;
    };
    std::vector<ViewLists> wl;
    int32_t *d_act_blk = nullptr, *d_act_lblk = nullptr, *d_act_sblk = nullptr, *d_act_win = nullptr;
    int32_t* d_flags = nullptr;
    BatchPlan plan;
    const void *schur_fn_plain = nullptr, *schur_fn_leangp = nullptr, *schur_fn_gen = nullptr;
    bool schur_pair_ok = false;
    static constexpr int kSchurPairBound = 384;
    int32_t* h_flags = nullptr;
    int rc = LIMO_OK;
    int n_slots = 0;
    int32_t* d_sched_ctl = nullptr;
    int shard_P = 1, shard_rank = 0;
    bool shard_virtual = true;
    std::vector<int> local_shards;
    std::vector<BatchView> pv;
    ExchangeLayout xl;
    double* arena_c = nullptr;
    std::vector<double*> blocks;
    std::vector<double*> trims;
    double* d_gather = nullptr;
    WinDesc* d_win_orig = nullptr;
    bool first_lin = false, assemble_pending = false;
    int64_t n_exchanges = 0, exchange_bytes = 0;
    double* d_lm_tmp = nullptr;
    std::vector<EventPair> ev_pool;
    size_t ev_used = 0;
    double k_ms_acc[2] = {0.0, 0.0};
    int64_t k_launches[2] = {0, 0};
    hipEvent_t ev_total_a = nullptr, ev_total_b = nullptr;
    double total_ms_acc = 0.0;
    double last_solve_sec = 0.0;
    int64_t n_rounds = 0, n_pair_launches = 0;
    int lin_variant = 1;

    ~limo_ba_batch() override {
        if (holds_pack_arena) ctx->pack_arena_busy = false;
        for (auto& a : allocs) ctx->pool_free(a.first, a.second);
        if (h_active) ctx->host_free(h_active, 64);
        if (h_flags) ctx->host_free(h_flags, h_flags_bytes);
        stream_teardown();
        for (auto& e : ev_pool) {
            (void)hipEventDestroy(e.a);
            (void)hipEventDestroy(e.b);
        }
        for (auto& e : act_ev)
            if (e) (void)hipEventDestroy(e);
        if (ev_total_a) (void)hipEventDestroy(ev_total_a);
        if (ev_total_b) (void)hipEventDestroy(ev_total_b);
    }

    int dmalloc(void** p, size_t bytes) {
        bytes = bytes ? bytes : 8;
        HIP_TRY(ctx, ctx->pool_alloc(p, bytes));
        allocs.push_back({*p, bytes});
        static const bool poison = std::getenv("KBA_POISON") != nullptr;
        if (poison) {
            HIP_TRY(ctx, hipMemsetAsync(*p, 0xFF, bytes, ctx->stream));
            HIP_TRY(ctx, hipStreamSynchronize(ctx->stream));
        }
        return LIMO_OK;
    }

    static const void* schur_kernel(int cls, int a, int b) {
        switch (cls * 100 + a * 10 + b) {
            case 14: return (const void*)k_schur_lean<1, false, 4>;
            case 23: return (const void*)k_schur_lean<2, false, 3>;
            case 113: return (const void*)k_schur_lean<1, true, 3>;
            case 122: return (const void*)k_schur_lean<2, true, 2>;
            case 132: return (const void*)k_schur_lean<3, true, 2>;
            case 210: return (const void*)k_schur_wide<1>;
            case 230: return (const void*)k_schur_wide<3>;
            case 260: return (const void*)k_schur_wide<6>;
            case 320: return (const void*)k_schur_wide<12>;
        }
        return nullptr;
    }

    int upload_list(const std::vector<int32_t>& v, const int32_t** out) {
        int32_t* d = nullptr;
        if (dmalloc((void**)&d, sizeof(int32_t) * std::max<size_t>(1, v.size()))) return LIMO_ERR_RUNTIME;
        if (!v.empty()) HIP_TRY(ctx, hipMemcpy(d, v.data(), sizeof(int32_t) * v.size(), hipMemcpyHostToDevice));
        *out = d;
        return LIMO_OK;
    }
    int build_full_sblk(size_t i) {
        WorkLists& f = wl[i].full;
        std::vector<int32_t> v;
        build_sblk_list(P, nullptr, c.schur_span, c.schur_span_gp, wl[i].owner, v, f.n_sblk_plain, f.n_sblk_fgp);
        f.n_sblk = (int)v.size();
        return upload_list(v, &f.sblk);
    }

    int upload() {
        std::memset(&bv, 0, sizeof(bv));
        int status = LIMO_OK;
        struct Ent {
            void** slot;
            size_t bytes, off;
            const void* init;
        };
        std::vector<Ent> ents;
        for_each_buffer(P, bv, [&](void** slot, size_t bytes, const void* init) { ents.push_back({slot, bytes ? bytes : 8, 0, init}); });
        st0.assign(P.n_win, WinState());
        std::memset(st0.data(), 0, sizeof(WinState) * st0.size());
        for (auto& q : st0) q.term = -1;
        for (Ent& e : ents)
            if (e.slot == (void**)&bv.st) e.init = st0.data();
        ents.push_back({(void**)&d_pose0, sizeof(double) * 7 * std::max(1, P.TK), 0, P.pose.empty() ? nullptr : P.pose.data()});
        ents.push_back({(void**)&d_pdir0, sizeof(double) * 3 * std::max(1, P.TK), 0, P.pdir.empty() ? nullptr : P.pdir.data()});
        ents.push_back({(void**)&d_pdist0, sizeof(double) * std::max(1, P.TK), 0, P.pdist.empty() ? nullptr : P.pdist.data()});
        ents.push_back({(void**)&d_lm0, sizeof(double) * 3 * std::max(1, P.TL), 0, P.lm.empty() ? nullptr : P.lm.data()});
        ents.push_back({(void**)&d_lm_state0, (size_t)std::max(1, P.TL), 0, P.lm_state.empty() ? nullptr : P.lm_state.data()});
        auto align = [](size_t x) { return (x + 255) / 256 * 256; };
        size_t init_total = 0, zero_total = 0;
        for (Ent& e : ents)
// ... 23 lines not shown
                const Ent* first = nullptr;
                for (size_t j = 0; j < i && !first; ++j)
                    if (ents[j].init == e.init && ents[j].bytes == e.bytes) first = &ents[j];
                if (first)
                    HIP_TRY(ctx, hipMemcpyAsync(arena + e.off, arena + first->off, e.bytes, hipMemcpyDeviceToDevice, ctx->stream));
                else
                    HIP_TRY(ctx, hipMemcpyAsync(arena + e.off, e.init, e.bytes, hipMemcpyHostToDevice, ctx->stream));
            }
        }
        if (zero_total) HIP_TRY(ctx, hipMemsetAsync(arena + init_total, 0, zero_total, ctx->stream));
        if (status != LIMO_OK) return status;
        pv.assign(1, bv);
        if (shard_P > 1) {
            xl = exchange_layout(P);
            d_win_orig = const_cast<WinDesc*>(bv.win);
            pv.assign(local_shards.size(), bv);
            auto zeros = [&](double** out, size_t n) -> int {
                if (dmalloc((void**)out, sizeof(double) * std::max<size_t>(1, n))) return LIMO_ERR_RUNTIME;
                HIP_TRY(ctx, hipMemsetAsync(*out, 0, sizeof(double) * std::max<size_t>(1, n), ctx->stream));
                return LIMO_OK;
            };
            if (zeros(&arena_c, xl.c_total)) return LIMO_ERR_RUNTIME;
            trims.assign(1 + local_shards.size(), nullptr);
            for (double*& t : trims)
                if (zeros(&t, xl.trim_count)) return LIMO_ERR_RUNTIME;
            blocks.assign(local_shards.size(), nullptr);
            if (!shard_virtual && zeros(&d_gather, (size_t)ctx->comm_world * xl.b_total)) return LIMO_ERR_RUNTIME;
            {
                std::vector<WinDesc> wc = exchange_consumer_windows(P);
                WinDesc* d_wc = nullptr;
                if (dmalloc((void**)&d_wc, sizeof(WinDesc) * wc.size())) return LIMO_ERR_RUNTIME;
                HIP_TRY(ctx, hipMemcpy(d_wc, wc.data(), sizeof(WinDesc) * wc.size(), hipMemcpyHostToDevice));
                exchange_bind_consumer(xl, bv, arena_c, trims[0], d_wc);
            }
            for (size_t i = 0; i < local_shards.size(); ++i) {
                if (zeros(&blocks[i], xl.b_total)) return LIMO_ERR_RUNTIME;
                exchange_bind_producer(xl, pv[i], blocks[i], trims[1 + i]);
                if (zeros(&pv[i].S_part, xl.spart_count)) return LIMO_ERR_RUNTIME;
            }
            if (!shard_virtual && dmalloc((void**)&d_lm_tmp, sizeof(double) * 3 * std::max(1, P.TL))) return LIMO_ERR_RUNTIME;
        }
        if (dmalloc((void**)&d_plane_rep, sizeof(double) * P.SO)) return LIMO_ERR_RUNTIME;
        if (dmalloc((void**)&d_plane_dep, sizeof(double) * P.SO)) return LIMO_ERR_RUNTIME;
        HIP_TRY(ctx, ctx->host_alloc((void**)&h_active, 64));
        HIP_TRY(ctx, hipHostGetDevicePointer((void**)&d_h_active, h_active, 0));
        bv.n_active_host = nullptr;
        h_flags_bytes = sizeof(int32_t) * std::max(1, P.n_win);
        HIP_TRY(ctx, ctx->host_alloc((void**)&h_flags, h_flags_bytes));
        if (dmalloc((void**)&d_act_blk, sizeof(int32_t) * std::max(1, P.n_blk))) return LIMO_ERR_RUNTIME;
        if (dmalloc((void**)&d_act_lblk, sizeof(int32_t) * std::max(1, P.n_lblk))) return LIMO_ERR_RUNTIME;
        if (dmalloc((void**)&d_act_sblk, sizeof(int32_t) * std::max(1, P.n_sblk))) return LIMO_ERR_RUNTIME;
        if (dmalloc((void**)&d_act_win, sizeof(int32_t) * std::max(1, P.n_win))) return LIMO_ERR_RUNTIME;
        if (dmalloc((void**)&d_flags, sizeof(int32_t) * std::max(1, P.n_win))) return LIMO_ERR_RUNTIME;
        wl.assign(pv.size(), ViewLists());
        for (size_t i = 0; i < wl.size(); ++i) {
            WorkLists& f = wl[i].full;
            f.n_blk = P.n_blk;
            f.n_lblk = P.n_lblk;
            f.n_win = P.n_win;
            if (shard_P == 1) continue;
            const int r = wl[i].owner = local_shards[i];
            auto owned = [&](const std::vector<int32_t>& owner, const int32_t** list, int* n) -> int {
                std::vector<int32_t> v;
                for (size_t k = 0; k < owner.size(); ++k)
                    if (owner[k] == r) v.push_back((int32_t)k);
                *n = (int)v.size();
                return upload_list(v, list);
            };
            if (owned(P.blk_owner, &f.blk, &f.n_blk) || owned(P.lblk_owner, &f.lblk, &f.n_lblk) || build_full_sblk(i)) return LIMO_ERR_RUNTIME;
        }
        plan = plan_batch(P, {schur_lean_lds_bytes, schur_wide_lds_bytes, lin_lm_lds_bytes(P.Vmax, true), kWideWaves, kTrimMaxSort});
        if (plan.wide_npw < 0) {
            ctx->err = "window with too many free camera slots for k_schur_wide";
            return LIMO_ERR_INVALID;
        }
        if (plan.any_fast) {
            schur_fn_plain = schur_kernel(0, plan.plain_tm, plan.plain_wpe);
            HIP_TRY(ctx, hipFuncSetAttribute(schur_fn_plain, hipFuncAttributeMaxDynamicSharedMemorySize, plan.plain_lds));
            schur_fn_leangp = schur_kernel(1, plan.gp_tm, plan.gp_wpe);
            HIP_TRY(ctx, hipFuncSetAttribute(schur_fn_leangp, hipFuncAttributeMaxDynamicSharedMemorySize, plan.leangp_lds));
            schur_pair_ok = plan.pair_ok && !(std::getenv("KBA_NO_SCHUR_PAIR") && std::atoi(std::getenv("KBA_NO_SCHUR_PAIR")) != 0);
            if (schur_pair_ok)
                HIP_TRY(ctx, hipFuncSetAttribute((const void*)k_schur_lean_pair<2, 3>, hipFuncAttributeMaxDynamicSharedMemorySize, std::max(plan.plain_lds, plan.leangp_lds)));
        }
        if (plan.any_gen) {
            schur_fn_gen = schur_kernel(2, plan.wide_npw, 0);
            HIP_TRY(ctx, hipFuncSetAttribute(schur_fn_gen, hipFuncAttributeMaxDynamicSharedMemorySize, plan.wide_lds));
        }
        HIP_TRY(ctx, hipFuncSetAttribute((const void*)k_cam_assemble, hipFuncAttributeMaxDynamicSharedMemorySize, plan.asm_bytes));
        HIP_TRY(ctx, hipFuncSetAttribute((const void*)k_cam_solve, hipFuncAttributeMaxDynamicSharedMemorySize, plan.solve_bytes));
        HIP_TRY(ctx, hipFuncSetAttribute((const void*)k_trim_select, hipFuncAttributeMaxDynamicSharedMemorySize, plan.trim_bytes));
        for (auto& e : act_ev) HIP_TRY(ctx, hipEventCreateWithFlags(&e, hipEventDisableTiming));
        HIP_TRY(ctx, hipEventCreate(&ev_total_a));
        HIP_TRY(ctx, hipEventCreate(&ev_total_b));
        return LIMO_OK;
    }

    bool spart_has_packed = false;
    bool pristine = true;
    int reset_state() {
        pristine = true;
        HIP_TRY(ctx, hipMemcpyAsync(bv.st, st0.data(), sizeof(WinState) * st0.size(), hipMemcpyHostToDevice, ctx->stream));
        HIP_TRY(ctx, hipMemcpyAsync(bv.pose, d_pose0, sizeof(double) * 7 * P.TK, hipMemcpyDeviceToDevice, ctx->stream));
        HIP_TRY(ctx, hipMemcpyAsync(bv.pdir, d_pdir0, sizeof(double) * 3 * P.TK, hipMemcpyDeviceToDevice, ctx->stream));
        HIP_TRY(ctx, hipMemcpyAsync(bv.pdist, d_pdist0, sizeof(double) * P.TK, hipMemcpyDeviceToDevice, ctx->stream));
        HIP_TRY(ctx, hipMemcpyAsync(bv.lm, d_lm0, sizeof(double) * 3 * P.TL, hipMemcpyDeviceToDevice, ctx->stream));
        HIP_TRY(ctx, hipMemcpyAsync(bv.lm_state, d_lm_state0, P.TL, hipMemcpyDeviceToDevice, ctx->stream));
        return LIMO_OK;
    }

    limo_ba_iteration* d_log = nullptr;
    int log_cap = 0;
    int log_alloc = 0;
    static int log_bound(const limo_ba_options& o) {
        const int64_t t = std::max(0, o.trim_solver_iterations), r = std::max(0, o.num_trim_rounds), m = std::max(0, o.max_num_iterations);
        return (int)std::min<int64_t>(r * ((t + 1) + (3 * t + 1)) + (m + 1), 1 << 24);
    }
    int bind_log(bool on) {
        const int cap = on ? log_bound(opts) : 0;
        if (!on && !log_cap) return LIMO_OK;
        if (cap > log_alloc) {
            if (dmalloc((void**)&d_log, sizeof(limo_ba_iteration) * (size_t)cap * (size_t)std::max(1, P.n_win))) return LIMO_ERR_RUNTIME;
            log_alloc = cap;
        }
        if (cap != log_cap) {
            HIP_TRY(ctx, hipStreamSynchronize(ctx->stream));
            for (int w = 0; w < P.n_win; ++w) {
                st0[w].log = on ? d_log + (size_t)w * cap : nullptr;
                st0[w].log_cap = cap;
            }
            log_cap = cap;
        }
        hipLaunchKernelGGL(k_log_bind, dim3(cdiv(P.n_win, 256)), dim3(256), 0, ctx->stream, bv, on ? d_log : (limo_ba_iteration*)nullptr, cap);
        HIP_TRY(ctx, hipGetLastError());
        return LIMO_OK;
    }
    int read_log(int w, int cap, limo_ba_iteration* out, int32_t* n) {
        *n = 0;
        if (!log_cap) return LIMO_OK;
        WinState s;
        HIP_TRY(ctx, hipMemcpyAsync(&s, bv.st + w, sizeof(WinState), hipMemcpyDeviceToHost, ctx->stream));
        HIP_TRY(ctx, hipStreamSynchronize(ctx->stream));
        const int have = std::max(0, std::min(s.log_n, log_cap)), m = std::min(have, cap);
        *n = have;
        if (m > 0) {
            HIP_TRY(ctx, hipMemcpyAsync(out, d_log + (size_t)w * log_cap, sizeof(limo_ba_iteration) * m, hipMemcpyDeviceToHost, ctx->stream));
            HIP_TRY(ctx, hipStreamSynchronize(ctx->stream));
        }
        return LIMO_OK;
    }
    int export_log() {
        ctx->last_log.clear();
        ctx->last_log_n.clear();
        ctx->last_log_off.clear();
        if (!log_cap) return LIMO_OK;
        std::vector<WinState> sv(P.n_win);
        HIP_TRY(ctx, hipMemcpyAsync(sv.data(), bv.st, sizeof(WinState) * sv.size(), hipMemcpyDeviceToHost, ctx->stream));
        HIP_TRY(ctx, hipStreamSynchronize(ctx->stream));
        size_t total = 0;
        for (int w = 0; w < P.n_win; ++w) {
            const int have = std::max(0, std::min(sv[w].log_n, log_cap));
            ctx->last_log_n.push_back(have);
            ctx->last_log_off.push_back(total);
            total += (size_t)have;
        }
        ctx->last_log.resize(total);
// ... 160 lines not shown
        if (ev_used == ev_pool.size()) {
            EventPair e;
            e.kernel = kernel;
            note(hipEventCreate(&e.a), "hipEventCreate");
            note(hipEventCreate(&e.b), "hipEventCreate");
            ev_pool.push_back(e);
        }
        EventPair* ep = &ev_pool[ev_used++];
        ep->kernel = kernel;
        note(hipEventRecord(ep->a, on ? on : ctx->stream), "hipEventRecord");
        return ep;
    }

    void linearize() override {
        hipStream_t s = ctx->stream;
        {
            if (P.TV) {
                hipLaunchKernelGGL(k_view_consts, dim3(cdiv(P.TV, 256)), dim3(256), 0, s, bv);
                LAUNCH_CHECK("k_view_consts");
            }
            EventPair* ep = timed(LIMO_KERNEL_LINEARIZE);
            for (size_t i = 0; i < pv.size(); ++i)
                if (wl[i].cur.n_lblk) {
                    launch_lin_lm(wl[i].cur.n_lblk, s, pv[i], wl[i].cur.lblk);
                    LAUNCH_CHECK("k_lin_lm");
                }
            if (ep) note(hipEventRecord(ep->b, s), "hipEventRecord");
        }
        if (shard_P > 1) {
            for (size_t i = 0; i < pv.size(); ++i)
                if (wl[i].cur.n_win) {
                    hipLaunchKernelGGL(k_shard_reduce, dim3(wl[i].cur.n_win), dim3(kBlock), 0, s, pv[i], wl[i].cur.win, local_shards[i], 0);
                    LAUNCH_CHECK("k_shard_reduce");
                }
            if (!first_lin) {
                assemble_pending = true;
                return;
            }
            first_lin = false;
            exchange(1);
        }
        assemble(it_no);
    }

    void assemble(int iter) {
        hipStream_t s = ctx->stream;
        const int slot = iter & 3;
        BatchView bvs = bv;
        bvs.n_active = bv.n_active + 2 * slot;
        bvs.n_active_host = d_h_active + slot;
        const WorkLists& a = wl[0].cur;
        launch_cam_assemble(bvs, a.win, a.n_win, s);
        LAUNCH_CHECK("k_cam_assemble");
        note(hipEventRecord(act_ev[slot], s), "record n_active");
    }

    int active_count() override {
        if (rc != LIMO_OK) return 0;
        const int cur = it_no++;
        if (cur == 0) return P.n_win;
        const int slot = (cur - 1) & 3;
        note(hipEventSynchronize(act_ev[slot]), "sync n_active");
        if (rc != LIMO_OK) return 0;
        const int a = h_active[slot], listed = wl[0].cur.n_win;
        static const bool trace = std::getenv("KBA_TRACE_ACTIVE") != nullptr;
        if (trace) std::fprintf(stderr, "[kba] iteration %d: active %d, listed %d, span %d\n", cur - 1, a, listed, c.schur_span);
        if (a > 0 && listed >= 8 && 2 * a <= listed) rebatch();
        return a;
    }

    void expire(int) override {
        if (assemble_pending) {
            assemble_pending = false;
            exchange(1);
            assemble(it_no - 1);
        }
        hipLaunchKernelGGL(k_expire, dim3(cdiv(P.n_win, 256)), dim3(256), 0, ctx->stream, bv);
        LAUNCH_CHECK("k_expire");
    }

    void launch_schur(const BatchView& v, const int32_t* wl_plain, int n_plain, const int32_t* wl_fgp, int n_fgp, const int32_t* wl_gen, int n_gen, bool pair,
                      hipStream_t s) {
        int span = c.schur_span, span_gp = c.schur_span_gp, packed = c.slab_packed;
        if (pair) {
            void* args[] = {(void*)&v, (void*)&wl_plain, (void*)&n_plain, (void*)&wl_fgp, (void*)&span, (void*)&span_gp, (void*)&packed};
            note(hipLaunchKernel((const void*)k_schur_lean_pair<2, 3>, dim3(n_plain + n_fgp), dim3(64), args, std::max(plan.plain_lds, plan.leangp_lds), s),
                 "launch k_schur_lean_pair");
            ++n_pair_launches;
        }
        if (!pair && n_plain) {
            void* args[] = {(void*)&v, (void*)&wl_plain, (void*)&span, (void*)&span_gp, (void*)&packed};
            note(hipLaunchKernel(schur_fn_plain, dim3(n_plain), dim3(64), args, plan.plain_lds, s), "launch k_schur_lean");
        }
        if (!pair && n_fgp) {
            void* args[] = {(void*)&v, (void*)&wl_fgp, (void*)&span, (void*)&span_gp, (void*)&packed};
            note(hipLaunchKernel(schur_fn_leangp, dim3(n_fgp), dim3(64), args, plan.leangp_lds, s), "launch k_schur_lean (gp)");
        }
        if (n_gen) {
            void* args[] = {(void*)&v, (void*)&wl_gen, (void*)&span, (void*)&span_gp};
            note(hipLaunchKernel(schur_fn_gen, dim3(n_gen), dim3(64 * kWideWaves), args, plan.wide_lds, s), "launch k_schur_wide");
        }
    }

    void launch_cam_assemble(const BatchView& v, const int32_t* list, int grid, hipStream_t s) {
        if (grid) hipLaunchKernelGGL(k_cam_assemble, dim3(grid), dim3(kBlock), plan.asm_bytes, s, v, c, list);
    }
    void launch_cam_solve(const BatchView& v, const int32_t* list, int grid, hipStream_t s) {
        if (grid) hipLaunchKernelGGL(k_cam_solve, dim3(grid), dim3(kBlock), plan.solve_bytes, s, v, c, list);
    }
    void launch_backsub(const BatchView& v, const int32_t* list, int grid, hipStream_t s) {
        if (grid) hipLaunchKernelGGL(k_backsub, dim3(grid), dim3(kBlock), 0, s, v, c, list);
    }
    void launch_step_decide(const BatchView& v, const int32_t* list, int grid, hipStream_t s) {
        if (grid) hipLaunchKernelGGL(k_step_decide, dim3(grid), dim3(64), 0, s, v, c, list);
    }
    void launch_after_step(const BatchView& v, const int32_t* list, int grid, hipStream_t s) {
        if (grid) hipLaunchKernelGGL(k_after_step, dim3(grid), dim3(kBlock), 0, s, v, c, list);
    }
    void launch_trim_residual(const BatchView& v, const int32_t* list, int grid, hipStream_t s) {
        if (grid) hipLaunchKernelGGL(k_trim_residual, dim3(grid), dim3(kBlock), 0, s, v, d_plane_rep, d_plane_dep, list);
    }
    void launch_trim_max(const BatchView& v, int shard, int grid, hipStream_t s) {
        if (grid) hipLaunchKernelGGL(k_trim_max, dim3(grid), dim3(kBlock), 0, s, v, (const double*)d_plane_rep, (const double*)d_plane_dep, shard, shard_P);
    }
    void launch_trim_select(const BatchView& v, int grid, hipStream_t s) {
        if (grid) hipLaunchKernelGGL(k_trim_select, dim3(grid), dim3(kBlock), plan.trim_bytes, s, v, c);
    }

    void step() override {
        hipStream_t s = ctx->stream;
        if (c.slab_packed) spart_has_packed = true;
        const WorkLists& a = wl[0].cur;
        {
            int n_schur = 0;
            for (size_t i = 0; i < pv.size(); ++i) n_schur += wl[i].cur.n_sblk;
            EventPair* ep = n_schur ? timed(LIMO_KERNEL_SCHUR) : nullptr;
            for (size_t i = 0; i < pv.size(); ++i) {
                const WorkLists& l = wl[i].cur;
                launch_schur(pv[i], l.sblk, l.n_sblk_plain, l.sblk + l.n_sblk_plain, l.n_sblk_fgp, l.sblk + l.n_sblk_plain + l.n_sblk_fgp,
                             l.n_sblk - l.n_sblk_plain - l.n_sblk_fgp, false, s);
                LAUNCH_CHECK("Schur kernels");
            }
            if (ep) note(hipEventRecord(ep->b, s), "hipEventRecord");
        }
        if (shard_P > 1) {
            if (a.n_win)
                for (size_t i = 0; i < pv.size(); ++i) {
                    hipLaunchKernelGGL(k_shard_reduce, dim3(a.n_win), dim3(kBlock), 0, s, pv[i], a.win, local_shards[i], 1);
                    hipLaunchKernelGGL(k_slab_reduce, dim3(a.n_win, 8), dim3(kBlock), 0, s, pv[i], a.win, shard_P);
                    LAUNCH_CHECK("k_slab_reduce");
                }
            if (assemble_pending) {
                assemble_pending = false;
                exchange(3);
                assemble(it_no - 1);
            } else {
                exchange(2);
            }
        }
        launch_cam_solve(bv, a.win, a.n_win, s);
        LAUNCH_CHECK("k_cam_solve");
        for (size_t i = 0; i < pv.size(); ++i) {
            launch_backsub(pv[i], wl[i].cur.lblk, wl[i].cur.n_lblk, s);
            LAUNCH_CHECK("k_backsub");
        }
        if (shard_P > 1 && a.n_win)
            for (size_t i = 0; i < pv.size(); ++i) {
                hipLaunchKernelGGL(k_shard_reduce, dim3(a.n_win), dim3(kBlock), 0, s, pv[i], a.win, local_shards[i], 2);
                LAUNCH_CHECK("k_shard_reduce");
            }
        exchange(4);
        launch_step_decide(bv, a.win, a.n_win, s);
        LAUNCH_CHECK("k_step_decide");
        for (size_t i = 0; i < pv.size(); ++i) {
            launch_after_step(pv[i], wl[i].cur.lblk, wl[i].cur.n_lblk, s);
            LAUNCH_CHECK("k_after_step");
        }
    }

// ... 386 lines not shown
        rc = pack_windows(n, windows, o, po, b->P, ctx->err);
    } catch (const std::bad_alloc&) {
        ctx->err = "pack_windows: out of host memory";
        return LIMO_ERR_RUNTIME;
    } catch (const std::exception& e) {
        ctx->err = std::string("pack_windows: ") + e.what();
        return LIMO_ERR_RUNTIME;
    }
    if (lending) {
        ctx->pack_arena_wanted = std::max(ctx->pack_arena_wanted, lend.wanted);
        if (lend.used > 0) {
            ctx->pack_arena_busy = true;
            b->holds_pack_arena = true;
        } else if (!ctx->pack_arena.p && lend.wanted > 0) {
            arena_resize(lend.wanted);
        }
    }
    const auto t_c1 = std::chrono::steady_clock::now();
    if (rc == LIMO_OK) {
        if (hipSetDevice(ctx->device) != hipSuccess) rc = LIMO_ERR_NO_DEVICE;
    }
    b->pose_batch = po.per_window_prior;
    b->shard_P = b->P.n_shards;
    b->shard_virtual = !shards_are_ranks;
    b->shard_rank = shards_are_ranks ? ctx->comm_rank : 0;
    if (b->shard_P > 1) {
        const int world = shards_are_ranks ? ctx->comm_world : 1, me = shards_are_ranks ? ctx->comm_rank : 0;
        for (int r = 0; r < b->shard_P; ++r)
            if (r % world == me) b->local_shards.push_back(r);
        if (b->local_shards.size() > 8) {
            ctx->err = "at most 8 shards per GPU";
            return LIMO_ERR_INVALID;
        }
    } else {
        b->local_shards.push_back(0);
    }
    b->c = b->consts_for(o);
    if (rc == LIMO_OK) rc = b->upload();
    if (std::getenv("KBA_PACK_TRACE"))
        std::fprintf(stderr, "[kba] create: pack %.1f ms, upload %.1f ms\n", std::chrono::duration<double, std::milli>(t_c1 - t_c0).count(),
                     std::chrono::duration<double, std::milli>(std::chrono::steady_clock::now() - t_c1).count());
    if (rc != LIMO_OK) return rc;
    *out = b.release();
    return LIMO_OK;
}

int limo_ba_batch_create(limo_ctx* ctx, int32_t n_windows, const limo_ba_window* windows, limo_ba_batch** out) {
    return batch_create_impl(ctx, n_windows, windows, nullptr, PackOptions(), out);
}

int limo_ba_batch_solve(limo_ba_batch* b, const limo_ba_options* opts) {
    if (!b) return LIMO_ERR_INVALID;
    limo_ctx* ctx = b->ctx;
    if (hipSetDevice(ctx->device) != hipSuccess) return LIMO_ERR_NO_DEVICE;
    if (opts) {
        if (opts->min_landmarks_for_trimming != b->opts.min_landmarks_for_trimming) {
            for (int w = 0; w < b->P.n_win; ++w) b->P.win[w].do_trim = b->P.win[w].n_lm > opts->min_landmarks_for_trimming;
            if (b->shard_P > 1) {
                const std::vector<WinDesc> wc = exchange_consumer_windows(b->P);
                HIP_TRY(ctx, hipMemcpy((void*)b->d_win_orig, b->P.win.data(), sizeof(WinDesc) * b->P.n_win, hipMemcpyHostToDevice));
                HIP_TRY(ctx, hipMemcpy((void*)b->bv.win, wc.data(), sizeof(WinDesc) * b->P.n_win, hipMemcpyHostToDevice));
            } else {
                HIP_TRY(ctx, hipMemcpyAsync((void*)b->bv.win, b->P.win.data(), sizeof(WinDesc) * b->P.n_win, hipMemcpyHostToDevice,
                                            ctx->stream));
            }
        }
        b->opts = *opts;
        b->c = b->consts_for(*opts);
    }
    b->rc = LIMO_OK;
    if (b->bind_log(ctx->iteration_log && b->shard_P == 1) != LIMO_OK) return LIMO_ERR_RUNTIME;
    const auto t0 = std::chrono::steady_clock::now();
    HIP_TRY(ctx, hipEventRecord(b->ev_total_a, ctx->stream));
    const SolveSwitches sw = read_solve_switches();
    SolveFacts facts;
    facts.max_solver_time_sec = b->opts.max_solver_time_sec;
    facts.shard_P = b->shard_P;
    facts.pose_batch = b->pose_batch;
    facts.pristine = b->pristine;
    facts.coop_strikes = ctx->coop_strikes;
    facts.coop_benched = ctx->coop_benched;
    const SolveChoice ch = choose_solve_path(b->P, b->plan, sw, facts);
    if (ch.benched) ++ctx->coop_benched;
    b->n_rounds = b->n_pair_launches = 0;
    b->lin_variant = 1;
    long long* info = ctx->last_solve_info;
    std::fill(info, info + 8, 0ll);
    auto launch_sequence = [&]() {
        info[0] = ch.fallback;
        if (ch.fallback == PATH_STREAMING)
            b->solve_streaming(sw);
        else
            run_schedule(*b, b->opts);
    };
    switch (ch.path) {
        case PATH_WG:
            info[0] = PATH_WG;
            b->solve_wg();
            break;
        case PATH_COOP:
            if (b->solve_coop(ch.coop, sw)) {
                info[0] = PATH_COOP;
                info[2] = ch.coop.G;
                ctx->coop_benched = 0;
                break;
            }
            [[fallthrough]];
        default:
            launch_sequence();
    }
    b->pristine = false;
    if (b->coop_launched) {
        b->coop_launched = false;
        HIP_TRY(ctx, hipStreamSynchronize(ctx->stream));
        if (b->h_active[8] == 0) ctx->coop_strikes = 0;
        if (b->h_active[8] != 0) {
            b->h_active[8] = 0;
            info[1] = 1;
            ++ctx->coop_fallbacks;
            ++ctx->coop_strikes;
            if (b->reset_state() != LIMO_OK) return LIMO_ERR_RUNTIME;
            b->rc = LIMO_OK;
            launch_sequence();
            b->pristine = false;
        }
    }
    if (b->shard_P > 1 && !b->shard_virtual) {
        hipLaunchKernelGGL(k_lm_owned, dim3(cdiv(b->P.TL, 256)), dim3(256), 0, ctx->stream, b->bv, b->d_lm_tmp, b->shard_rank, b->shard_P,
                           ctx->comm_world);
        if (ctx->xfn) {
            b->host_exchange(b->d_lm_tmp, b->bv.lm, (size_t)3 * b->P.TL, 1);
            if (b->rc != LIMO_OK) return b->rc;
        } else {
            const ncclResult_t r = ncclAllReduce(b->d_lm_tmp, b->bv.lm, (size_t)3 * b->P.TL, ncclDouble, ncclSum, (ncclComm_t)ctx->comm, ctx->stream);
            b->note_nccl(r, "ncclAllReduce(landmarks)");
            if (r != ncclSuccess) return b->rc;
        }
        ++b->n_exchanges;
        b->exchange_bytes += (int64_t)sizeof(double) * 3 * b->P.TL;
    }
    if (info[0] == PATH_STREAMING) {
        info[3] = (long long)b->groups.size();
        info[4] = b->n_slots;
    }
    info[5] = b->n_rounds;
    info[6] = b->n_pair_launches;
    info[7] = b->lin_variant;
    HIP_TRY(ctx, hipEventRecord(b->ev_total_b, ctx->stream));
    HIP_TRY(ctx, hipStreamSynchronize(ctx->stream));
    float ms = 0.f;
    HIP_TRY(ctx, hipEventElapsedTime(&ms, b->ev_total_a, b->ev_total_b));
    b->total_ms_acc += ms;
    b->last_solve_sec = std::chrono::duration<double>(std::chrono::steady_clock::now() - t0).count();
    return b->rc;
}

int limo_ba_batch_reset(limo_ba_batch* b) {
    if (!b) return LIMO_ERR_INVALID;
    if (hipSetDevice(b->ctx->device) != hipSuccess) return LIMO_ERR_NO_DEVICE;
    return b->reset_state();
}

int limo_ba_batch_download(limo_ba_batch* b, limo_ba_window* windows_out, limo_ba_report* reports) {
    if (!b) return LIMO_ERR_INVALID;
    limo_ctx* ctx = b->ctx;
    const PackedBatch& P = b->P;
    std::vector<double> pose_v, pdir_v, pdist_v, lm_v;
    std::vector<WinState> st_v;
    const double *pose = nullptr, *pdir = nullptr, *pdist = nullptr, *lm = nullptr;
    const WinState* st = nullptr;
    {
        const char* lo = reinterpret_cast<const char*>(b->bv.st);
        const char* hi = reinterpret_cast<const char*>(b->bv.lm) + sizeof(double) * 3 * (size_t)P.TL;
        auto inside = [&](const void* q) { return reinterpret_cast<const char*>(q) >= lo && reinterpret_cast<const char*>(q) < hi; };
        const bool neighbours = hi > lo && inside(b->bv.pose) && inside(b->bv.pdir) && inside(b->bv.pdist) && (P.TL == 0 || inside(b->bv.lm));
        const size_t span = neighbours ? (size_t)(hi - lo) : 0;
        void* hbuf = nullptr;
        if (neighbours && span <= ctx->staging.cap && ctx->staging.p) {
            hbuf = ctx->staging.p;
        } else if (neighbours && span <= limo_ctx::kBigStageMax) {
            if (ctx->staging_big.ensure(span, span + span / 4, limo_ctx::kBigStageMax) == hipSuccess)
                hbuf = ctx->staging_big.p;
            else
                (void)hipGetLastError();
        }
        if (hbuf) {
            HIP_TRY(ctx, hipMemcpyAsync(hbuf, lo, span, hipMemcpyDeviceToHost, ctx->stream));
            HIP_TRY(ctx, hipStreamSynchronize(ctx->stream));
            const char* h = static_cast<const char*>(hbuf);
            auto at = [&](const void* q) { return h + (reinterpret_cast<const char*>(q) - lo); };
            st = reinterpret_cast<const WinState*>(at(b->bv.st));
            pose = reinterpret_cast<const double*>(at(b->bv.pose));
            pdir = reinterpret_cast<const double*>(at(b->bv.pdir));
            pdist = reinterpret_cast<const double*>(at(b->bv.pdist));
            lm = reinterpret_cast<const double*>(at(b->bv.lm));
        } else {
            pose_v.resize((size_t)P.TK * 7);
            pdir_v.resize((size_t)P.TK * 3);
            pdist_v.resize(P.TK);
            lm_v.resize((size_t)P.TL * 3);
            st_v.resize(P.n_win);
            HIP_TRY(ctx, hipMemcpyAsync(pose_v.data(), b->bv.pose, sizeof(double) * pose_v.size(), hipMemcpyDeviceToHost, ctx->stream));
            HIP_TRY(ctx, hipMemcpyAsync(pdir_v.data(), b->bv.pdir, sizeof(double) * pdir_v.size(), hipMemcpyDeviceToHost, ctx->stream));
            HIP_TRY(ctx, hipMemcpyAsync(pdist_v.data(), b->bv.pdist, sizeof(double) * pdist_v.size(), hipMemcpyDeviceToHost, ctx->stream));
            if (P.TL) HIP_TRY(ctx, hipMemcpyAsync(lm_v.data(), b->bv.lm, sizeof(double) * lm_v.size(), hipMemcpyDeviceToHost, ctx->stream));
            HIP_TRY(ctx, hipMemcpyAsync(st_v.data(), b->bv.st, sizeof(WinState) * st_v.size(), hipMemcpyDeviceToHost, ctx->stream));
            HIP_TRY(ctx, hipStreamSynchronize(ctx->stream));
            pose = pose_v.data();
            pdir = pdir_v.data();
            pdist = pdist_v.data();
            lm = lm_v.data();
            st = st_v.data();
        }
    }
    if (windows_out)
        for (int w = 0; w < P.n_win; ++w)
            if (windows_out[w].n_kf != P.win[w].n_kf || windows_out[w].n_lm != P.win[w].n_lm) {
                ctx->err = "download: window shape differs from create()";
                return LIMO_ERR_INVALID;
            }
    auto one_window = [&](int w) {
        const WinDesc& d = P.win[w];
        if (windows_out) {
            limo_ba_window& W = windows_out[w];
            std::memcpy(W.kf_pose, pose + 7 * (size_t)d.kf0, sizeof(double) * 7 * d.n_kf);
            std::memcpy(W.kf_plane_dir, pdir + 3 * (size_t)d.kf0, sizeof(double) * 3 * d.n_kf);
            std::memcpy(W.kf_plane_dist, pdist + d.kf0, sizeof(double) * d.n_kf);
            for (int l = 0; l < d.n_lm; ++l)
                std::memcpy(W.lm_pos + 3 * (size_t)P.lm_id[d.lm0 + l], lm + 3 * (size_t)(d.lm0 + l), sizeof(double) * 3);
        }
// ... 113 lines not shown
    ctx->comm_world = world;
    return LIMO_OK;
}

int limo_ctx_comm_init_host(limo_ctx* ctx, limo_exchange_fn fn, void* user, int rank, int world) {
    if (!ctx || (fn && (world < 1 || rank < 0 || rank >= world))) return LIMO_ERR_INVALID;
    if (ctx->comm) {
        (void)ncclCommDestroy((ncclComm_t)ctx->comm);
        ctx->comm = nullptr;
    }
    ctx->xfn = fn;
    ctx->xuser = user;
    ctx->comm_rank = fn ? rank : 0;
    ctx->comm_world = fn ? world : 1;
    return LIMO_OK;
}

int limo_ba_solve_sharded(limo_ctx* ctx, limo_ba_window* window, const limo_ba_options* opts, int n_shards,
                          limo_ba_report* report) {
    if (!ctx || !window) return LIMO_ERR_INVALID;
    const bool ranks = ctx->has_transport();
    if (n_shards < 1 || (ranks && n_shards % ctx->comm_world != 0) || n_shards > 8 * (ranks ? ctx->comm_world : 1)) {
        ctx->err = "limo_ba_solve_sharded: n_shards must be a multiple of the communicator size, at most 8 shards per GPU";
        return LIMO_ERR_INVALID;
    }
    PackOptions po;
    po.shards = n_shards;
    limo_ba_batch* b = nullptr;
    ctx->last_log.clear();
    ctx->last_log_n.clear();
    ctx->last_log_off.clear();
    int rc = batch_create_impl(ctx, 1, window, opts, po, &b, ranks);
    if (rc != LIMO_OK) return rc;
    rc = limo_ba_batch_solve(b, opts);
    limo_ba_report rep;
    if (rc == LIMO_OK) rc = limo_ba_batch_download(b, window, &rep);
    if (rc == LIMO_OK && report) *report = rep;
    ctx->exchange_stats[0] = b->n_exchanges;
    ctx->exchange_stats[1] = b->exchange_bytes;
    ctx->exchange_stats[2] = rc == LIMO_OK ? rep.iterations_total : 0;
    limo_ba_batch_destroy(b);
    return rc;
}

static int solve_n(limo_ctx* ctx, int32_t n, limo_ba_window* windows, const limo_ba_options* opts, const PackOptions& po, limo_ba_report* reports,
                   const char* what) {
    using Clock = std::chrono::steady_clock;
    static const bool trace = std::getenv("KBA_HOST_TRACE") != nullptr;
    const auto t_a = Clock::now();
    limo_ba_batch* b = nullptr;
    int rc = batch_create_impl(ctx, n, windows, opts, po, &b);
    if (rc != LIMO_OK) return rc;
    const auto t0 = Clock::now();
    rc = limo_ba_batch_solve(b, nullptr);
    const auto t1 = Clock::now();
    if (rc == LIMO_OK) rc = limo_ba_batch_download(b, windows, reports);
    {
        const int lrc = b->export_log();
        if (rc == LIMO_OK) rc = lrc;
    }
    const auto t2 = Clock::now();
    if (reports)
        for (int w = 0; w < n; ++w) reports[w].time_sec = std::chrono::duration<double>(t2 - t0).count();
    limo_ba_batch_destroy(b);
    if (trace) {
        auto us = [](Clock::time_point a, Clock::time_point c) { return std::chrono::duration<double, std::micro>(c - a).count(); };
        std::fprintf(stderr, "[kba] %s (%d windows): create %.0f us, solve %.0f us, download %.0f us, destroy %.0f us\n", what, (int)n, us(t_a, t0), us(t0, t1),
                     us(t1, t2), us(t2, Clock::now()));
    }
    return rc;
}

int64_t limo_ctx_coop_fallbacks(const limo_ctx* ctx) { return ctx ? (int64_t)ctx->coop_fallbacks : 0; }

int limo_ctx_exchange_stats(limo_ctx* ctx, int64_t* stats3) {
    if (!ctx || !stats3) return LIMO_ERR_INVALID;
    for (int i = 0; i < 3; ++i) stats3[i] = ctx->exchange_stats[i];
    return LIMO_OK;
}

int limo_ctx_last_solve_info(const limo_ctx* ctx, int64_t info[8]) {
    if (!ctx || !info) return LIMO_ERR_INVALID;
    for (int i = 0; i < 8; ++i) info[i] = ctx->last_solve_info[i];
    return LIMO_OK;
}

int limo_ctx_set_iteration_log(limo_ctx* ctx, int32_t on) {
    if (!ctx) return LIMO_ERR_INVALID;
    ctx->iteration_log = on != 0;
    return LIMO_OK;
}

static const char* iteration_log_args(int32_t window, int32_t n_win, int32_t cap, const limo_ba_iteration* out, const int32_t* n) {
    if (!n) return "n is NULL";
    if (cap < 0) return "cap < 0";
    if (cap > 0 && !out) return "out is NULL with cap > 0";
    if (window < 0 || (n_win >= 0 && window >= n_win)) return "window out of range";
    return nullptr;
}

int limo_ba_batch_iteration_log(limo_ba_batch* b, int32_t window, int32_t cap, limo_ba_iteration* out, int32_t* n) {
    if (!b) return LIMO_ERR_INVALID;
    limo_ctx* ctx = b->ctx;
    if (const char* bad = iteration_log_args(window, b->P.n_win, cap, out, n)) {
        ctx->err = std::string("limo_ba_batch_iteration_log: ") + bad;
        return LIMO_ERR_INVALID;
    }
    if (hipSetDevice(ctx->device) != hipSuccess) return LIMO_ERR_NO_DEVICE;
    return b->read_log(window, cap, out, n);
}

int limo_ctx_last_iteration_log(limo_ctx* ctx, int32_t window, int32_t cap, limo_ba_iteration* out, int32_t* n) {
    if (!ctx) return LIMO_ERR_INVALID;
    const int32_t n_win = ctx->last_log_n.empty() ? -1 : (int32_t)ctx->last_log_n.size();
    if (const char* bad = iteration_log_args(window, n_win, cap, out, n)) {
        ctx->err = std::string("limo_ctx_last_iteration_log: ") + bad;
        return LIMO_ERR_INVALID;
    }
    *n = 0;
    if (n_win < 0) return LIMO_OK;
    *n = ctx->last_log_n[window];
    const int m = std::min(*n, cap);
    if (m > 0) std::memcpy(out, ctx->last_log.data() + ctx->last_log_off[window], sizeof(limo_ba_iteration) * m);
    return LIMO_OK;
}

int limo_ba_solve(limo_ctx* ctx, limo_ba_window* window, const limo_ba_options* opts, limo_ba_report* report) {
    if (!ctx || !window) return LIMO_ERR_INVALID;
    return solve_n(ctx, 1, window, opts, PackOptions(), report, "limo_ba_solve");
}

int limo_ba_solve_fixed_landmarks(limo_ctx* ctx, limo_ba_window* window, const uint8_t* lm_fixed, const limo_ba_options* opts,
                                  limo_ba_report* report) {
    if (!ctx || !window) return LIMO_ERR_INVALID;
    PackOptions po;
    po.lm_fixed = lm_fixed ? &lm_fixed : nullptr;
    return solve_n(ctx, 1, window, opts, po, report, "limo_ba_solve_fixed_landmarks");
}

int limo_ba_batch_create_fixed_landmarks(limo_ctx* ctx, int32_t n_windows, const limo_ba_window* windows, const uint8_t* const* lm_fixed,
                                         limo_ba_batch** out) {
    PackOptions po;
    po.lm_fixed = lm_fixed;
    return batch_create_impl(ctx, n_windows, windows, nullptr, po, out);
}

int limo_ba_adjust_pose_only(limo_ctx* ctx, limo_ba_window* window, const limo_speed_prior* prior,
                             const limo_ba_options* opts, limo_ba_report* report) {
    if (!ctx || !window) return LIMO_ERR_INVALID;
    PackOptions po;
    po.pose_only = true;
    po.prior = prior;
    return solve_n(ctx, 1, window, opts, po, report, "limo_ba_adjust_pose_only");
}

int limo_ba_batch_create_pose_only(limo_ctx* ctx, int32_t n_windows, const limo_ba_window* windows, const limo_speed_prior* priors,
                                   limo_ba_batch** out) {
    PackOptions po;
    po.pose_only = true;
    po.per_window_prior = true;
    po.window_priors = priors;
    return batch_create_impl(ctx, n_windows, windows, nullptr, po, out);
}

int limo_ba_adjust_pose_only_batch(limo_ctx* ctx, int32_t n_windows, limo_ba_window* windows, const limo_speed_prior* priors,
                                   const limo_ba_options* opts, limo_ba_report* reports) {
// ... 148 lines not shown
```

Measured before the change: 38130 windows/s.

## Classify ground-plane Schur groups and use a narrow two-panel tile when possible

At pack time, each ground-plane Schur group is classified by whether its plane-related columns come from a single keyframe with a contiguous column span. Groups that qualify are routed to a new NARROW variant of the lean Schur kernel. It accumulates only the camera columns plus that span (two 16-wide panels instead of three) and scatters the result into the packed slab, explicitly zeroing the uncovered entries. This is meant to cut the arithmetic, shared-memory use and accumulator registers of the ground-plane Schur assembly. The cost is per-group dispatch branching inside one kernel, added classification work on the host, and correctness risk in the index remapping and zero-fill.

```diff
diff --git a/include/limo_hip.h b/include/limo_hip.h
--- a/include/limo_hip.h
+++ b/include/limo_hip.h
@@ -125,6 +125,7 @@
 int limo_ctx_exchange_stats(limo_ctx* ctx, int64_t* stats3);
 int64_t limo_ctx_coop_fallbacks(const limo_ctx* ctx);
 int limo_ctx_last_solve_info(const limo_ctx* ctx, int64_t info[8]);
+int limo_ctx_last_schur_gp_info(const limo_ctx* ctx, int64_t info[4]);
 
 typedef struct limo_ba_iteration {
     int32_t solve;
diff --git a/limo_amd/_ffi.py b/limo_amd/_ffi.py
--- a/limo_amd/_ffi.py
+++ b/limo_amd/_ffi.py
@@ -279,6 +279,7 @@
     "limo_ctx_exchange_stats",
     "limo_ctx_coop_fallbacks",
     "limo_ctx_last_solve_info",
+    "limo_ctx_last_schur_gp_info",
     "limo_ctx_set_iteration_log",
     "limo_ba_batch_iteration_log",
     "limo_ctx_last_iteration_log",
@@ -407,6 +408,8 @@
     lib.limo_ctx_coop_fallbacks.restype = C.c_int64
     if hasattr(lib, "limo_ctx_last_solve_info"):
         lib.limo_ctx_last_solve_info.argtypes = [vp, c_int64_p]
+    if hasattr(lib, "limo_ctx_last_schur_gp_info"):
+        lib.limo_ctx_last_schur_gp_info.argtypes = [vp, c_int64_p]
     if hasattr(lib, "limo_ctx_set_iteration_log"):
         lib.limo_ctx_set_iteration_log.argtypes = [vp, C.c_int32]
         lib.limo_ba_batch_iteration_log.argtypes = [vp, C.c_int32, C.c_int32, C.POINTER(BaIteration), c_int32_p]
diff --git a/limo_amd/ba.py b/limo_amd/ba.py
--- a/limo_amd/ba.py
+++ b/limo_amd/ba.py
@@ -82,6 +82,11 @@
         _check(self.lib.limo_ctx_last_solve_info(self.ptr, v), self.ptr, "limo_ctx_last_solve_info")
         keys = ("recovered", "coop_G", "groups", "slots", "rounds", "pair_launches", "lin_variant")
         return dict({"path": self.SOLVE_PATHS.get(int(v[0]), "NONE")}, **{k: int(v[1 + i]) for i, k in enumerate(keys)})
+
+    def last_schur_gp_info(self):
+        v = (C.c_int64 * 4)()
+        _check(self.lib.limo_ctx_last_schur_gp_info(self.ptr, v), self.ptr, "limo_ctx_last_schur_gp_info")
+        return dict(zip(("narrow_groups", "wide_groups", "narrow_launches", "wide_launches"), (int(x) for x in v)))
 
     def set_iteration_log(self, on):
         _check(self.lib.limo_ctx_set_iteration_log(self.ptr, int(bool(on))), self.ptr, "limo_ctx_set_iteration_log")
diff --git a/limo_amd/csrc/kba_batch_plan.hpp b/limo_amd/csrc/kba_batch_plan.hpp
--- a/limo_amd/csrc/kba_batch_plan.hpp
+++ b/limo_amd/csrc/kba_batch_plan.hpp
@@ -27,6 +27,7 @@
     int asm_bytes = 0, solve_bytes = 0, trim_bytes = 0;
     int schur_wave_lds = 0;
     int onelaunch_lds = 0;
+    bool narrow = false;
 };
 
 inline BatchPlan plan_batch(const PackedBatch& P, const PlanKernelSizes& ks) {
@@ -54,6 +55,7 @@
         p.gp_wpe = p.gp_tm == 1 ? 3 : 2;
         p.leangp_lds = ks.lean_lds(max_nf + 1);
         p.pair_ok = p.plain_tm == 2 && p.gp_tm == 3;
+        p.narrow = p.gp_tm == 3 && P.n_sgrp_narrow > 0;
     }
     if (p.any_gen) {
         const int tiles = t_gen * (t_gen + 1) / 2, npw = (tiles + ks.wide_waves - 1) / ks.wide_waves;
@@ -115,6 +117,7 @@
     double coop_timeout_ms = 50.0;
     bool groups_set = false;
     int groups = 0;
+    bool gp_wide = false;
 };
 
 inline SolveSwitches read_solve_switches() {
@@ -135,6 +138,7 @@
         s.groups_set = true;
         s.groups = std::atoi(e);
     }
+    s.gp_wide = on("KBA_SCHUR_GP_WIDE");
     return s;
 }
 
diff --git a/limo_amd/csrc/kba_items.hpp b/limo_amd/csrc/kba_items.hpp
--- a/limo_amd/csrc/kba_items.hpp
+++ b/limo_amd/csrc/kba_items.hpp
@@ -609,8 +609,16 @@
 KBA_HD int64_t slab_packed_base(int q, int n_plain, int nf, int nfq) {
     return q < n_plain ? (int64_t)q * schur_need_pad(nfq) : (int64_t)n_plain * schur_need_pad(nfq) + (int64_t)(q - n_plain) * schur_need_pad(nf);
 }
+template <class Windows>
+inline int schur_gp_panels(const Windows& win) {
+    int max_nf = 0;
+    for (const WinDesc& d : win)
+        if (d.schur_fast && d.nf > max_nf) max_nf = d.nf;
+    const int t = (max_nf + 16) / 16;
+    return t < 3 ? t : 3;
+}
 KBA_HD SchurGroup schur_group_make(const WinDesc& wd, int w, int sb, int span, int span_gp, const int32_t* sblk_lm0, const int32_t* sblk_n,
-                                   const int32_t* cslot) {
+                                   const int32_t* cslot, const int32_t* lm_gp = nullptr, const int32_t* gp_kf = nullptr) {
     SchurGroup g;
     const int sb_last = schur_group_last(wd, sb, span, span_gp);
     g.w = w;
@@ -620,14 +628,44 @@
     g.nf = wd.nf, g.nfq = wd.nfq, g.nf_pad = wd.nf_pad;
     g.kf0 = wd.kf0, g.view0 = wd.view0, g.cam0 = wd.cam0;
     g.q_slab = schur_slab_of(wd, sb, span, span_gp);
-    g.pad = 0;
     for (int k = 0; k < 4; ++k) {
         const bool on = k < wd.n_fk;
         g.kl[k] = on ? wd.fk[k] : -1;
         g.view[k] = on ? wd.fk_view[k] : -1;
         const int ci = on ? cslot[wd.cam0 + wd.fk[k] * kCamSlots] : -1;
         g.col0[k] = ci < 0 ? -1 : schur_col(ci, wd.nfq);
-        g.pad2[k] = 0;
+    }
+    g.gp_class = kSchurGpWide;
+    g.gp_ci0 = g.gp_ns = 0;
+    g.pad2[0] = g.pad2[1] = 0;
+    if (lm_gp && gp_kf && sb - wd.sblk0 >= wd.n_sblk_plain) {
+        int kn = kSchurGpNoPlane;
+        bool narrow = true;
+        for (int l = 0; l < g.n_lm && narrow; ++l) {
+            const int gr = lm_gp[g.lm_first + l];
+            if (gr < 0) continue;
+            const int k = gp_kf[gr] - wd.kf0;
+            const int32_t* cs = cslot + wd.cam0 + k * kCamSlots;
+            if (cs[6] < 0 && cs[7] < 0 && cs[8] < 0 && cs[9] < 0) continue;
+            if (cs[0] < 0 || (kn >= 0 && kn != k)) narrow = false;
+            kn = k;
+        }
+        if (narrow && kn >= 0) {
+            int first = -1, n = 0;
+            for (int s = 6; s < kCamSlots; ++s) {
+                const int ci = cslot[wd.cam0 + kn * kCamSlots + s];
+                if (ci < 0) continue;
+                if (first < 0) first = ci;
+                if (ci != first + n) narrow = false;
+                ++n;
+            }
+            g.gp_ci0 = first, g.gp_ns = n;
+        }
+        if (narrow) {
+            g.gp_class = kn;
+        } else {
+            g.gp_ci0 = g.gp_ns = 0;
+        }
     }
     g.off_tile = wd.spart_off + (int64_t)g.q_slab * ((int64_t)wd.nf_pad * wd.nf_pad);
     g.off_packed = wd.spart_off + slab_packed_base(g.q_slab, schur_plain_slabs(wd, span), wd.nf, wd.nfq);
@@ -645,6 +683,12 @@
     if (zr == nfq) return schur_need_index(n, zc - 1, n);
     return schur_need_index(n, zr - (zr > nfq ? 1 : 0), zc - (zc > nfq ? 1 : 0));
 }
+KBA_HD int schur_narrow_col(int zc, int nfq, int ci0, int ns) {
+    if (zc <= nfq) return zc;
+    return zc - 1 >= ci0 && zc - 1 < ci0 + ns ? nfq + 1 + (zc - 1 - ci0) : -1;
+}
+KBA_HD int schur_narrow_zc(int c, int nfq, int ci0) { return c <= nfq ? c : c - nfq + ci0; }
+KBA_HD bool schur_narrow_covers(int ci, int nfq, int ci0, int ns) { return ci < nfq || (ci >= ci0 && ci < ci0 + ns); }
 
 struct LogProd {
     double m;
diff --git a/limo_amd/csrc/kba_kernels.hip b/limo_amd/csrc/kba_kernels.hip
--- a/limo_amd/csrc/kba_kernels.hip
+++ b/limo_amd/csrc/kba_kernels.hip
@@ -671,8 +671,9 @@
         __syncthreads();
     }
 }
-template <int TM, bool GP, bool COOP>
+template <int TM, bool GP, bool COOP, bool NARROW = false>
 __device__ __forceinline__ void schur_lean_group(const BatchView& bv, int sb, int span, int span_gp, int slab_packed, double* smem) {
+    static_assert(!NARROW || (TM == 2 && GP && !COOP), "the narrow tile: two panels, ground-plane groups, packed slabs");
     SchurGroup g;
     if (span == kSchurSpan && span_gp == kSchurSpanGp) {
         g = bv.sgrp[sb];
@@ -680,9 +681,12 @@
         const int w = bv.sblk_win[sb];
         g = schur_group_make(bv.win[w], w, sb, span, span_gp, bv.sblk_lm0, bv.sblk_n, bv.cslot);
     }
+    if constexpr (NARROW) {
+        if (g.gp_class == kSchurGpWide) return;
+    }
     const int active = COOP ? 1 : __hip_atomic_load(&bv.st[g.w].active, __ATOMIC_RELAXED, __HIP_MEMORY_SCOPE_AGENT);
     const int nfq = g.nfq, nfp = g.nf_pad;
-    const int ncol = GP ? g.nf + 1 : nfq + 1;
+    const int ncol = NARROW ? nfq + 1 + g.gp_ns : GP ? g.nf + 1 : nfq + 1;
     const int ld = schur_lean_ld(ncol);
     const int Tt = (ncol + 15) / 16;
     constexpr bool kTT = !GP && TM == 2;
@@ -781,7 +785,8 @@
             if (li >= 5 && li < 15) mine_w[li == 14 ? kSpQq1 : li - 5] = vw ? v2 : 0.0;
             if (li < kCamSlots) {
                 mine_w[kSpScale + li] = sc;
-                zcs[kq * 12 + li] = ci < 0 ? -1 : schur_col(ci, nfq);
+                const int zc = ci < 0 ? -1 : schur_col(ci, nfq);
+                zcs[kq * 12 + li] = NARROW ? schur_narrow_col(zc, nfq, g.gp_ci0, g.gp_ns) : zc;
             }
         }
         if (lane < 16) Z[3 * kSchurLm * ld + lane] = 0.0;
@@ -933,6 +938,34 @@
     const bool packed = !COOP && slab_packed != 0;
     double* out = bv.S_part + (packed ? g.off_packed : g.off_tile);
     const int T = nfp / 16;
+    if constexpr (NARROW) {
+        double* outn = bv.S_part + g.off_packed;
+        const int nf = g.nf, ci0 = g.gp_ci0, ns = g.gp_ns;
+        int idx = 0;
+#pragma unroll
+        for (int tr = 0; tr < 2; ++tr)
+#pragma unroll
+            for (int tc = tr; tc < 2; ++tc) {
+                if (tc < Tt) {
+#pragma unroll
+                    for (int r = 0; r < 4; ++r) {
+                        const int row = tr * 16 + kq + 4 * r, col = tc * 16 + li;
+                        if (row < ncol && col < ncol) {
+                            const int k = slab_packed_write(true, schur_narrow_zc(row, nfq, ci0), schur_narrow_zc(col, nfq, ci0), nf, nfq);
+                            if (k >= 0) outn[k] = acc[idx][r];
+                        }
+                    }
+                }
+                ++idx;
+            }
+        for (int ca = kq; ca < nf; ca += 4) {
+            const int cb = nfq + li;
+            if (cb >= ca && cb < nf && !(schur_narrow_covers(ca, nfq, ci0, ns) && schur_narrow_covers(cb, nfq, ci0, ns)))
+                outn[schur_need_index(nf, ca, cb)] = 0.0;
+        }
+        if (nfq + lane < nf && !schur_narrow_covers(nfq + lane, nfq, ci0, ns)) outn[schur_need_index(nf, nfq + lane, nf)] = 0.0;
+        return;
+    }
     if (two_tile && packed) {
 #pragma unroll
         for (int r = 0; r < 4; ++r) {
@@ -1046,8 +1079,17 @@
     extern __shared__ __attribute__((aligned(16))) double smem[];
     schur_lean_group<TM, GP, false>(bv, sb, span, span_gp, slab_packed, smem);
 }
-
-template <int TMP, int TMG>
+__global__ __launch_bounds__(64) __attribute__((amdgpu_waves_per_eu(2, 2))) void k_schur_lean_gp(BatchView bv, const int32_t* wl) {
+    const int sb = wl_at(bv, wl, blockIdx.x);
+    if (sb < 0) return;
+    extern __shared__ __attribute__((aligned(16))) double smem[];
+    if (bv.sgrp[sb].gp_class != kSchurGpWide)
+        schur_lean_group<2, true, false, true>(bv, sb, kSchurSpan, kSchurSpanGp, 1, smem);
+    else
+        schur_lean_group<3, true, false>(bv, sb, kSchurSpan, kSchurSpanGp, 1, smem);
+}
+
+template <int TMP, int TMG, bool NARROW = false>
 __global__ __launch_bounds__(64) void k_schur_lean_pair(BatchView bv, const int32_t* wl_plain, int n_plain_cap, const int32_t* wl_gp, int span, int span_gp, int slab_packed) {
     extern __shared__ __attribute__((aligned(16))) double smem[];
     if ((int)blockIdx.x < n_plain_cap) {
@@ -1055,7 +1097,11 @@
         if (sb >= 0) schur_lean_group<TMP, false, false>(bv, sb, span, span_gp, slab_packed, smem);
     } else {
         const int sb = wl_at(bv, wl_gp, blockIdx.x - n_plain_cap);
-        if (sb >= 0) schur_lean_group<TMG, true, false>(bv, sb, span, span_gp, slab_packed, smem);
+        if (sb < 0) return;
+        if (NARROW && bv.sgrp[sb].gp_class != kSchurGpWide)
+            schur_lean_group<2, true, false, true>(bv, sb, span, span_gp, slab_packed, smem);
+        else
+            schur_lean_group<TMG, true, false>(bv, sb, span, span_gp, slab_packed, smem);
     }
 }
 
diff --git a/limo_amd/csrc/kba_layout.hpp b/limo_amd/csrc/kba_layout.hpp
--- a/limo_amd/csrc/kba_layout.hpp
+++ b/limo_amd/csrc/kba_layout.hpp
@@ -70,15 +70,17 @@
     int32_t nf, nfq, nf_pad;
     int32_t kf0, view0, cam0;
     int32_t q_slab;
-    int32_t pad;
+    int32_t gp_class;
     int32_t kl[4];
     int32_t view[4];
     int32_t col0[4];
     int64_t off_tile;
     int64_t off_packed;
-    int32_t pad2[4];
+    int32_t gp_ci0, gp_ns;
+    int32_t pad2[2];
 };
 static_assert(sizeof(SchurGroup) == 128, "one cache line per record");
+constexpr int kSchurGpNoPlane = -1, kSchurGpWide = -2;
 
 struct WinState {
     int32_t active, need_lin, first, accept;
diff --git a/limo_amd/csrc/kba_pack.cpp b/limo_amd/csrc/kba_pack.cpp
--- a/limo_amd/csrc/kba_pack.cpp
+++ b/limo_amd/csrc/kba_pack.cpp
@@ -754,12 +754,20 @@
     P.n_lblk = (int)P.lblk_win.size();
     P.n_sblk = (int)P.sblk_win.size();
     P.sgrp.assign((size_t)P.n_sblk, SchurGroup{});
+    const bool classify = schur_gp_panels(P.win) >= 3;
     for_windows([&](int w) {
         const WinDesc& d = P.win[w];
         if (!d.schur_fast) return;
         for (int sb = d.sblk0; sb < d.sblk0 + d.n_sblk; ++sb)
-            P.sgrp[sb] = schur_group_make(d, w, sb, kSchurSpan, kSchurSpanGp, P.sblk_lm0.data(), P.sblk_n.data(), P.cslot.data());
+            P.sgrp[sb] = schur_group_make(d, w, sb, kSchurSpan, kSchurSpanGp, P.sblk_lm0.data(), P.sblk_n.data(), P.cslot.data(),
+                                          classify ? P.lm_gp.data() : nullptr, classify ? P.gp_kf.data() : nullptr);
     });
+    P.n_sgrp_narrow = P.n_sgrp_wide = 0;
+    if (classify)
+        for (const WinDesc& d : P.win) {
+            if (!d.schur_fast) continue;
+            for (int i = d.n_sblk_plain; i < d.n_sblk; i += kSchurSpanGp) (P.sgrp[d.sblk0 + i].gp_class == kSchurGpWide ? P.n_sgrp_wide : P.n_sgrp_narrow)++;
+        }
     if (P.evaluate_only) {
         P.echunk.clear();
         P.obs_rank.assign((size_t)std::max(1, P.TO), -1);
diff --git a/limo_amd/csrc/kba_pack.hpp b/limo_amd/csrc/kba_pack.hpp
--- a/limo_amd/csrc/kba_pack.hpp
+++ b/limo_amd/csrc/kba_pack.hpp
@@ -85,6 +85,7 @@
     uvec<int32_t> obs_src;
     std::vector<int32_t> lblk_win, lblk_lm0, lblk_n, sblk_win, sblk_lm0, sblk_n;
     std::vector<SchurGroup> sgrp;
+    int32_t n_sgrp_narrow = 0, n_sgrp_wide = 0;
     std::vector<int32_t> gp_lm, gp_kf;
     std::vector<double> gp_w;
 };
diff --git a/limo_amd/csrc/limo_ctx.hpp b/limo_amd/csrc/limo_ctx.hpp
--- a/limo_amd/csrc/limo_ctx.hpp
+++ b/limo_amd/csrc/limo_ctx.hpp
@@ -48,6 +48,7 @@
     int coop_strikes = 0;
     int coop_benched = 0;
     long long last_solve_info[8] = {0, 0, 0, 0, 0, 0, 0, 0};
+    long long last_schur_gp_info[4] = {0, 0, 0, 0};
     bool iteration_log = false;
     std::vector<limo_ba_iteration> last_log;
     std::vector<int32_t> last_log_n;
diff --git a/limo_amd/csrc/limo_hip.hip b/limo_amd/csrc/limo_hip.hip
--- a/limo_amd/csrc/limo_hip.hip
+++ b/limo_amd/csrc/limo_hip.hip
@@ -76,6 +76,8 @@
     int32_t* d_flags = nullptr;
     BatchPlan plan;
     const void *schur_fn_plain = nullptr, *schur_fn_leangp = nullptr, *schur_fn_gen = nullptr;
+    const void* schur_fn_narrow = nullptr;
+    bool gp_wide = false;
     bool schur_pair_ok = false;
     static constexpr int kSchurPairBound = 384;
     int32_t* h_flags = nullptr;
@@ -103,6 +105,7 @@
     double total_ms_acc = 0.0;
     double last_solve_sec = 0.0;
     int64_t n_rounds = 0, n_pair_launches = 0;
+    int64_t n_narrow_launches = 0, n_widegp_launches = 0;
     int lin_variant = 1;
 
     ~limo_ba_batch() override {
@@ -292,6 +295,12 @@
             schur_pair_ok = plan.pair_ok && !(std::getenv("KBA_NO_SCHUR_PAIR") && std::atoi(std::getenv("KBA_NO_SCHUR_PAIR")) != 0);
             if (schur_pair_ok)
                 HIP_TRY(ctx, hipFuncSetAttribute((const void*)k_schur_lean_pair<2, 3>, hipFuncAttributeMaxDynamicSharedMemorySize, std::max(plan.plain_lds, plan.leangp_lds)));
+            if (plan.narrow) {
+                schur_fn_narrow = (const void*)k_schur_lean_gp;
+                HIP_TRY(ctx, hipFuncSetAttribute(schur_fn_narrow, hipFuncAttributeMaxDynamicSharedMemorySize, plan.leangp_lds));
+                if (schur_pair_ok)
+                    HIP_TRY(ctx, hipFuncSetAttribute((const void*)k_schur_lean_pair<2, 3, true>, hipFuncAttributeMaxDynamicSharedMemorySize, std::max(plan.plain_lds, plan.leangp_lds)));
+            }
         }
         if (plan.any_gen) {
             schur_fn_gen = schur_kernel(2, plan.wide_npw, 0);
@@ -618,9 +627,12 @@
     void launch_schur(const BatchView& v, const int32_t* wl_plain, int n_plain, const int32_t* wl_fgp, int n_fgp, const int32_t* wl_gen, int n_gen, bool pair,
                       hipStream_t s) {
         int span = c.schur_span, span_gp = c.schur_span_gp, packed = c.slab_packed;
+        const bool narrow = plan.narrow && !gp_wide && packed && span == kSchurSpan && span_gp == kSchurSpanGp;
+        const bool wide = !narrow || P.n_sgrp_wide > 0;
         if (pair) {
             void* args[] = {(void*)&v, (void*)&wl_plain, (void*)&n_plain, (void*)&wl_fgp, (void*)&span, (void*)&span_gp, (void*)&packed};
-            note(hipLaunchKernel((const void*)k_schur_lean_pair<2, 3>, dim3(n_plain + n_fgp), dim3(64), args, std::max(plan.plain_lds, plan.leangp_lds), s),
+            note(hipLaunchKernel(narrow ? (const void*)k_schur_lean_pair<2, 3, true> : (const void*)k_schur_lean_pair<2, 3>, dim3(n_plain + n_fgp), dim3(64), args,
+                                 std::max(plan.plain_lds, plan.leangp_lds), s),
                  "launch k_schur_lean_pair");
             ++n_pair_launches;
         }
@@ -628,9 +640,17 @@
             void* args[] = {(void*)&v, (void*)&wl_plain, (void*)&span, (void*)&span_gp, (void*)&packed};
             note(hipLaunchKernel(schur_fn_plain, dim3(n_plain), dim3(64), args, plan.plain_lds, s), "launch k_schur_lean");
         }
-        if (!pair && n_fgp) {
+        if (!pair && n_fgp && narrow) {
+            void* args[] = {(void*)&v, (void*)&wl_fgp};
+            note(hipLaunchKernel(schur_fn_narrow, dim3(n_fgp), dim3(64), args, plan.leangp_lds, s), "launch k_schur_lean_gp");
+        }
+        if (!pair && n_fgp && !narrow) {
             void* args[] = {(void*)&v, (void*)&wl_fgp, (void*)&span, (void*)&span_gp, (void*)&packed};
             note(hipLaunchKernel(schur_fn_leangp, dim3(n_fgp), dim3(64), args, plan.leangp_lds, s), "launch k_schur_lean (gp)");
+        }
+        if (pair || n_fgp) {
+            n_narrow_launches += narrow ? 1 : 0;
+            n_widegp_launches += wide ? 1 : 0;
         }
         if (n_gen) {
             void* args[] = {(void*)&v, (void*)&wl_gen, (void*)&span, (void*)&span_gp};
@@ -1183,7 +1203,8 @@
     facts.coop_benched = ctx->coop_benched;
     const SolveChoice ch = choose_solve_path(b->P, b->plan, sw, facts);
     if (ch.benched) ++ctx->coop_benched;
-    b->n_rounds = b->n_pair_launches = 0;
+    b->n_rounds = b->n_pair_launches = b->n_narrow_launches = b->n_widegp_launches = 0;
+    b->gp_wide = sw.gp_wide;
     b->lin_variant = 1;
     long long* info = ctx->last_solve_info;
     std::fill(info, info + 8, 0ll);
@@ -1247,6 +1268,10 @@
     info[5] = b->n_rounds;
     info[6] = b->n_pair_launches;
     info[7] = b->lin_variant;
+    ctx->last_schur_gp_info[0] = b->P.n_sgrp_narrow;
+    ctx->last_schur_gp_info[1] = b->P.n_sgrp_wide;
+    ctx->last_schur_gp_info[2] = b->n_narrow_launches;
+    ctx->last_schur_gp_info[3] = b->n_widegp_launches;
     HIP_TRY(ctx, hipEventRecord(b->ev_total_b, ctx->stream));
     HIP_TRY(ctx, hipStreamSynchronize(ctx->stream));
     float ms = 0.f;
@@ -1526,6 +1551,12 @@
 int limo_ctx_last_solve_info(const limo_ctx* ctx, int64_t info[8]) {
     if (!ctx || !info) return LIMO_ERR_INVALID;
     for (int i = 0; i < 8; ++i) info[i] = ctx->last_solve_info[i];
+    return LIMO_OK;
+}
+
+int limo_ctx_last_schur_gp_info(const limo_ctx* ctx, int64_t info[4]) {
+    if (!ctx || !info) return LIMO_ERR_INVALID;
+    for (int i = 0; i < 4; ++i) info[i] = ctx->last_schur_gp_info[i];
     return LIMO_OK;
 }
 
```

After: 38680 windows/s, median of 6. +1.4%, better.
